# Young768/KungFu

Hardware: AMD Instinct MI355X
Metric: images/sec/GPU ResNet-50 SynchronousSGD at 1/2/4/8 MI355X; scaling efficiency (higher is better)
Workload: dtype bf16

## Files before the change

### csrc/kernels/bind_bn.cpp

```cpp
#include "bind_util.hpp"

#include <vector>

using namespace kfb;

namespace {

const auto kCL = at::MemoryFormat::ChannelsLast;

kfk::BNShape bn_shape(const at::Tensor &x, const char *op) {
    check_cl4(x, op, "x", kAnyGpu);
    const int C = narrow(x.size(1), op, "x");
    TORCH_CHECK(kfk::bn_supported_channels(C), op, ": unsupported channel count ", C);
    return kfk::BNShape{x.numel() / C, C};
}

struct BNCommon {
    float *rm = nullptr, *rv = nullptr;
    int64_t *nbt = nullptr;
};

BNCommon bn_common(const char *op, int C, const Dev &dev, const at::Tensor &weight, const at::Tensor &bias,
                   const OptTensor &running_mean, const OptTensor &running_var, const OptTensor &num_batches,
                   bool training) {
    check_dense(weight, op, "weight", dev, at::kFloat, C);
    check_dense(bias, op, "bias", dev, at::kFloat, C);
    BNCommon b;
    if (has(running_mean)) {
        TORCH_CHECK(has(running_var), op, ": running_var missing");
        b.rm = running_mean->data_ptr<float>();
        b.rv = running_var->data_ptr<float>();
    }
    TORCH_CHECK(training || b.rm, op, ": eval mode needs running stats");
    if (training && has(num_batches)) {
        TORCH_CHECK(num_batches->scalar_type() == at::kLong && num_batches->numel() == 1 && num_batches->is_cuda(),
                    op, ": num_batches_tracked must be a 1-element int64 GPU tensor");
        b.nbt = num_batches->data_ptr<int64_t>();
    }
    return b;
}

at::Tensor bn_dy(at::Tensor dy, const at::Tensor &x, int C, int64_t *ld) {
    *ld = 0;
    if (dy.is_contiguous(kCL)) return dy;
    const int64_t s3 = dy.stride(3);
    const bool slice = dy.stride(1) == 1 && s3 >= C && s3 % 8 == 0 && dy.stride(2) == dy.size(3) * s3 &&
                       dy.stride(0) == dy.size(2) * dy.size(3) * s3 &&
                       reinterpret_cast<uintptr_t>(dy.data_ptr()) % 16 == 0;
    if (!slice) return dy.contiguous(kCL);
    *ld = s3;
    return dy;
}

void check_bn_dy(const at::Tensor &dy, const at::Tensor &x, const char *op) {
    TORCH_CHECK(dy.scalar_type() == at::kBFloat16 && dy.sizes() == x.sizes() && dy.device() == x.device(), op,
                ": dy must be a bf16 tensor of x's shape on its device");
}

std::vector<std::vector<at::Tensor>> bn_finalize_multi(std::vector<at::Tensor> xs, std::vector<at::Tensor> sums,
                                                       std::vector<at::Tensor> weights, std::vector<at::Tensor> biases,
                                                       std::vector<OptTensor> running_means,
                                                       std::vector<OptTensor> running_vars,
                                                       std::vector<OptTensor> num_batches,
                                                       std::vector<double> momentum, std::vector<double> eps) {
    const char *op = "bn_finalize_multi";
    const size_t n = xs.size();
    TORCH_CHECK(n >= 1 && n <= static_cast<size_t>(kfk::kBnFinMax) && sums.size() == n && weights.size() == n &&
                    biases.size() == n && running_means.size() == n && running_vars.size() == n &&
                    num_batches.size() == n && momentum.size() == n && eps.size() == n,
                "bn_finalize_multi: 1..8 BNs, every list of the same length");
    kfk::BnFinBatch b{};
    b.n = static_cast<int>(n);
    for (size_t i = 0; i < n; ++i) {
        auto sh = bn_shape(xs[i], op);
        const Dev dev = xs[0].device();
        TORCH_CHECK(xs[i].device() == *dev, "bn_finalize_multi: xs must be on one device");
        auto c = bn_common(op, sh.channels, dev, weights[i], biases[i], running_means[i], running_vars[i],
                           num_batches[i], true);
        kfk::BnFinDesc &d = b.d[i];
        TORCH_CHECK(sums[i].defined(), "bn_finalize_multi: sums must be defined");
        d.sums = stats_ptr(sums[i], op, sh.channels, dev, "sums");
        d.gamma = weights[i].data_ptr<float>(), d.beta = biases[i].data_ptr<float>();
        d.run_mean = c.rm, d.run_var = c.rv, d.nbt = c.nbt;
        d.rows = sh.rows, d.C = sh.channels;
        d.momentum = static_cast<float>(momentum[i]), d.eps = static_cast<float>(eps[i]);
    }
    std::vector<std::vector<at::Tensor>> out;
    for (size_t i = 0; i < n; ++i) {
        kfk::BnFinDesc &d = b.d[i];
        auto fopt = xs[i].options().dtype(at::kFloat);
        at::Tensor mean = at::empty({d.C}, fopt), invstd = at::empty({d.C}, fopt), coef = at::empty({2 * d.C}, fopt);
        d.mean = mean.data_ptr<float>(), d.invstd = invstd.data_ptr<float>(), d.coef = coef.data_ptr<float>();
        out.push_back({mean, invstd, coef});
    }
    c10::DeviceGuard gd(xs[0].device());
    kfk::launch_bn_sums_finalize_multi(b, stream_of(xs[0], 0));
    return out;
}

std::vector<at::Tensor> bn_forward(at::Tensor x, OptTensor res, at::Tensor weight, at::Tensor bias,
                                   OptTensor running_mean, OptTensor running_var, double momentum, double eps,
                                   bool training, bool relu, OptTensor num_batches, OptTensor sums, OptTensor res_coef,
                                   bool apply, OptTensor out, c10::optional<std::vector<at::Tensor>> pre) {
    const char *op = "bn_forward";
    auto sh = bn_shape(x, op);
    const int C = sh.channels;
    const Dev dev = x.device();
    auto b = bn_common(op, C, dev, weight, bias, running_mean, running_var, num_batches, training);
    const uint16_t *rp = nullptr;
    if (has(res)) {
        check_cl4(*res, op, "res", dev, x.sizes());
        rp = bf16(*res);
    }
    const float *rc = nullptr;
    if (has(res_coef)) {
        TORCH_CHECK(rp, "bn_forward: res_coef (the residual BN's f32 [scale(C); shift(C)]) needs res");
        check_dense(*res_coef, op, "res_coef", dev, at::kFloat, 2 * C);
        rc = res_coef->data_ptr<float>();
    }
    int64_t y_ld = 0;
    if (has(out)) {
        TORCH_CHECK(apply && !rp && relu && out->scalar_type() == at::kBFloat16 && out->sizes() == x.sizes() &&
                        out->stride(1) == 1 && out->stride(3) >= C && out->stride(3) % 8 == 0 &&
                        out->stride(2) == out->size(3) * out->stride(3) &&
                        out->stride(0) == out->size(2) * out->stride(2) &&
                        reinterpret_cast<uintptr_t>(out->data_ptr()) % 16 == 0 && out->device() == x.device(),
                    "bn_forward: out must be a 16-byte aligned channel slice of a channels_last bf16 tensor "
                    "(BN+ReLU, no residual)");
        y_ld = out->stride(3);
    }
    const bool prefin = pre.has_value();
    if (prefin) {
        TORCH_CHECK(pre->size() == 3 && training && has(sums), "bn_forward: pre must be (mean, invstd, coef) with sums");
        check_dense((*pre)[0], op, "pre[0]", dev, at::kFloat, C);
        check_dense((*pre)[1], op, "pre[1]", dev, at::kFloat, C);
        check_dense((*pre)[2], op, "pre[2]", dev, at::kFloat, 2 * C);
    }
    double *sp = training ? stats_ptr(sums, op, C, dev, "sums") : nullptr;

    c10::DeviceGuard gd(x.device());
    auto fopt = x.options().dtype(at::kFloat);
    at::Tensor y;
    if (has(out)) y = *out;
    else if (apply) y = at::empty_like(x, kCL);
    at::Tensor mean, invstd, coef;
    if (prefin) mean = (*pre)[0], invstd = (*pre)[1], coef = (*pre)[2];
    else mean = at::empty({C}, fopt), invstd = at::empty({C}, fopt), coef = at::empty({2 * C}, fopt);
    at::Tensor mask;
    if (apply && rp && relu) mask = at::empty({sh.rows * (C / 8)}, x.options().dtype(at::kByte));
    at::Tensor partial;
    if (training && !sp) partial = at::empty({2 * static_cast<int64_t>(kfk::bn_num_chunks(sh)) * C}, fopt);
    kfk::launch_bn_forward(bf16(x), rp, weight.data_ptr<float>(), bias.data_ptr<float>(),
                           apply ? bf16_mut(y) : nullptr, mask.defined() ? mask.data_ptr<uint8_t>() : nullptr, sh, relu,
                           training, b.rm, b.rv, static_cast<float>(momentum), static_cast<float>(eps),
                           partial.defined() ? partial.data_ptr<float>() : nullptr, mean.data_ptr<float>(),
                           invstd.data_ptr<float>(), coef.data_ptr<float>(), b.nbt, stream_of(x, 0), sp, rc, apply, y_ld,
                           prefin);
    return {y, mean, invstd, coef, mask};
}

std::vector<at::Tensor> bn_backward(at::Tensor dy, at::Tensor x, at::Tensor mean, at::Tensor invstd, at::Tensor weight,
                                    at::Tensor fcoef, OptTensor mask, bool relu, bool training, bool want_dres,
                                    OptTensor sums, OptTensor dres_x, OptTensor dres_sums) {
    const char *op = "bn_backward";
    auto sh = bn_shape(x, op);
    const int C = sh.channels;
    const Dev dev = x.device();
    check_bn_dy(dy, x, op);
    check_dense(mean, op, "mean", dev, at::kFloat, C);
    check_dense(invstd, op, "invstd", dev, at::kFloat, C);
    check_dense(weight, op, "weight", dev, at::kFloat, C);
    check_dense(fcoef, op, "fcoef", dev, at::kFloat, 2 * C);
    const uint8_t *mp = nullptr;
    if (has(mask)) {
        check_dense(*mask, op, "mask", dev, at::kByte, sh.rows * (C / 8));
        mp = mask->data_ptr<uint8_t>();
    }
    double *sp = stats_ptr(sums, op, C, dev, "sums");
    const uint16_t *dsx = nullptr;
    double *dsp = nullptr;
    if (has(dres_x)) {
        TORCH_CHECK(want_dres && has(dres_sums),
                    "bn_backward: dres_x (second BN's input) needs want_dres and its f64 sums workspace dres_sums");
        check_cl4(*dres_x, op, "dres_x", dev, x.sizes());
        dsx = bf16(*dres_x);
        dsp = stats_ptr(dres_sums, op, C, dev, "dres_sums");
    }
    c10::DeviceGuard gd(x.device());
    int64_t dy_ld;
    dy = bn_dy(dy, x, C, &dy_ld);
    auto fopt = x.options().dtype(at::kFloat);
    auto dx = at::empty_like(x, kCL);
    at::Tensor dres;
    if (want_dres) dres = at::empty_like(x, kCL);
    at::Tensor dw = at::empty({C}, fopt), db = at::empty({C}, fopt), coef = at::empty({3 * C}, fopt);
    at::Tensor partial;
    if (!sp) partial = at::empty({2 * static_cast<int64_t>(kfk::bn_num_chunks(sh)) * C}, fopt);
    kfk::launch_bn_backward(bf16(dy), bf16(x), fcoef.data_ptr<float>(), mp, mean.data_ptr<float>(),
                            invstd.data_ptr<float>(), weight.data_ptr<float>(), sh, relu, training,
                            partial.defined() ? partial.data_ptr<float>() : nullptr, dw.data_ptr<float>(),
                            db.data_ptr<float>(), coef.data_ptr<float>(), bf16_mut(dx),
                            want_dres ? bf16_mut(dres) : nullptr, stream_of(x, 0), sp, dsx, dsp, dy_ld);
    return {dx, dres, dw, db};
}

std::vector<std::vector<at::Tensor>> bn_backward_multi(std::vector<at::Tensor> dys, std::vector<at::Tensor> xs,
                                                       std::vector<at::Tensor> means, std::vector<at::Tensor> invstds,
                                                       std::vector<at::Tensor> weights, std::vector<at::Tensor> fcoefs) {
    const char *op = "bn_backward_multi";
    const size_t n = xs.size();
    TORCH_CHECK(n >= 1 && n <= static_cast<size_t>(kfk::kBnFinMax) && dys.size() == n && means.size() == n &&
                    invstds.size() == n && weights.size() == n && fcoefs.size() == n,
                "bn_backward_multi: 1..8 BNs, every list of the same length");
    struct Piece {
        at::Tensor dy, dx, dw, db, coef, partial;
        int64_t ld;
        kfk::BNShape sh;
    };
    std::vector<Piece> ps(n);
    const Dev dev = xs[0].device();
    for (size_t i = 0; i < n; ++i) {
        ps[i].sh = bn_shape(xs[i], op);
        const int C = ps[i].sh.channels;
        TORCH_CHECK(xs[i].device() == *dev, "bn_backward_multi: xs must be on one device");
        check_bn_dy(dys[i], xs[i], op);
        check_dense(fcoefs[i], op, "fcoefs", dev, at::kFloat, 2 * C);
        check_dense(means[i], op, "means", dev, at::kFloat, C);
        check_dense(invstds[i], op, "invstds", dev, at::kFloat, C);
        check_dense(weights[i], op, "weights", dev, at::kFloat, C);
    }
    c10::DeviceGuard gd(xs[0].device());
    kfk::BnBwdFinBatch fb{};
    fb.n = static_cast<int>(n);
    for (size_t i = 0; i < n; ++i) {
        Piece &p = ps[i];
        const int C = p.sh.channels;
        p.dy = bn_dy(dys[i], xs[i], C, &p.ld);
        auto fopt = xs[i].options().dtype(at::kFloat);
        p.dx = at::empty_like(xs[i], kCL);
        p.dw = at::empty({C}, fopt), p.db = at::empty({C}, fopt), p.coef = at::empty({3 * C}, fopt);
        p.partial = at::empty({2 * static_cast<int64_t>(kfk::bn_num_chunks(p.sh)) * C}, fopt);
        kfk::BnBwdFinDesc &d = fb.d[i];
        d.partial = p.partial.data_ptr<float>();
        d.nchunks = kfk::bn_num_chunks(p.sh), d.C = C, d.rows = p.sh.rows;
        d.gamma = weights[i].data_ptr<float>(), d.mean = means[i].data_ptr<float>(), d.invstd = invstds[i].data_ptr<float>();
        d.dgamma = p.dw.data_ptr<float>(), d.dbeta = p.db.data_ptr<float>(), d.coef = p.coef.data_ptr<float>();
    }
    const hipStream_t st = stream_of(xs[0], 0);
    for (int phase : {1, 2}) {
        if (phase == 2) kfk::launch_bn_bwd_finalize_multi(fb, st);
        for (size_t i = 0; i < n; ++i) {
            Piece &p = ps[i];
            kfk::launch_bn_backward(bf16(p.dy), bf16(xs[i]), fcoefs[i].data_ptr<float>(), nullptr,
                                    means[i].data_ptr<float>(), invstds[i].data_ptr<float>(),
                                    weights[i].data_ptr<float>(), p.sh, true, true, p.partial.data_ptr<float>(),
                                    p.dw.data_ptr<float>(), p.db.data_ptr<float>(), p.coef.data_ptr<float>(),
                                    bf16_mut(p.dx), nullptr, st, nullptr, nullptr, nullptr, p.ld, phase);
        }
    }
    std::vector<std::vector<at::Tensor>> out;
    for (auto &p : ps) out.push_back({p.dx, p.dw, p.db});
    return out;
}

std::vector<at::Tensor> bn_pool_forward(at::Tensor x, at::Tensor weight, at::Tensor bias, OptTensor running_mean,
                                        OptTensor running_var, double momentum, double eps, bool training,
                                        OptTensor num_batches, OptTensor sums) {
    const char *op = "bn_pool_forward";
    auto sh = bn_shape(x, op);
    const int C = sh.channels;
    const Dev dev = x.device();
    const int H = narrow(x.size(2), op, "x"), W = narrow(x.size(3), op, "x");
    TORCH_CHECK(kfk::bn_pool_supported(sh, H, W), "bn_pool_forward: unsupported shape");
    double *sp = training ? stats_ptr(sums, op, C, dev, "sums") : nullptr;
    auto b = bn_common(op, C, dev, weight, bias, running_mean, running_var, num_batches, training);
    c10::DeviceGuard gd(x.device());
    auto fopt = x.options().dtype(at::kFloat);
    const int OH = kfk::pool_out(H), OW = kfk::pool_out(W);
    auto yp = at::empty({x.size(0), C, OH, OW}, x.options().memory_format(kCL));
    auto arg = at::empty({x.size(0) * OH * OW * C}, x.options().dtype(at::kByte));
    auto mean = at::empty({C}, fopt), invstd = at::empty({C}, fopt), coef = at::empty({2 * C}, fopt);
    at::Tensor partial, xarg;
    if (training) {
        partial = at::empty({2 * static_cast<int64_t>(kfk::bn_num_chunks(sh)) * C}, fopt);
        xarg = at::empty_like(yp, kCL);
    }
    kfk::launch_bn_pool_forward(bf16(x), weight.data_ptr<float>(), bias.data_ptr<float>(), bf16_mut(yp),
                                arg.data_ptr<uint8_t>(), sh, H, W, training, b.rm, b.rv, static_cast<float>(momentum),
                                static_cast<float>(eps), training ? partial.data_ptr<float>() : nullptr,
                                mean.data_ptr<float>(), invstd.data_ptr<float>(), coef.data_ptr<float>(), b.nbt,
                                stream_of(x, 0), sp, xarg.defined() ? bf16_mut(xarg) : nullptr);
    return {yp, mean, invstd, coef, arg, xarg};
}

std::vector<at::Tensor> bn_pool_backward(at::Tensor dyp, at::Tensor arg, at::Tensor x, at::Tensor mean,
                                         at::Tensor invstd, at::Tensor weight, at::Tensor fcoef, bool training,
                                         OptTensor xarg, bool apply) {
    const char *op = "bn_pool_backward";
    auto sh = bn_shape(x, op);
    const int C = sh.channels;
    const Dev dev = x.device();
    const int H = narrow(x.size(2), op, "x"), W = narrow(x.size(3), op, "x");
    const int64_t psz[4] = {x.size(0), C, kfk::pool_out(H), kfk::pool_out(W)};
    TORCH_CHECK(dyp.scalar_type() == at::kBFloat16 && dyp.sizes() == at::IntArrayRef(psz) && dyp.device() == x.device(),
                "bn_pool_backward: dy must be the pooled [N, C, PH, PW] bf16 gradient on x's device");
    check_dense(arg, op, "arg", dev, at::kByte, dyp.numel());
    check_dense(mean, op, "mean", dev, at::kFloat, C);
    check_dense(invstd, op, "invstd", dev, at::kFloat, C);
    check_dense(weight, op, "weight", dev, at::kFloat, C);
    check_dense(fcoef, op, "fcoef", dev, at::kFloat, 2 * C);
    const bool pooled = training && has(xarg);
    if (pooled) check_cl4(*xarg, op, "xarg", dev, psz);
    c10::DeviceGuard gd(x.device());
    if (!dyp.is_contiguous(kCL)) dyp = dyp.contiguous(kCL);
    auto fopt = x.options().dtype(at::kFloat);
    auto dx = apply ? at::empty_like(x, kCL) : at::empty({0}, x.options());
    auto dw = at::empty({C}, fopt), db = at::empty({C}, fopt), coef = at::empty({3 * C}, fopt);
    auto partial = at::empty({2 * static_cast<int64_t>(kfk::bn_num_chunks(sh)) * C}, fopt);
    at::Tensor sums;
    if (pooled) sums = at::zeros({2 * C * kfk::kStatSlots}, x.options().dtype(at::kDouble));
    kfk::launch_bn_pool_backward(bf16(dyp), arg.data_ptr<uint8_t>(), bf16(x), fcoef.data_ptr<float>(),
                                 mean.data_ptr<float>(), invstd.data_ptr<float>(), weight.data_ptr<float>(), sh, H, W,
                                 training, partial.data_ptr<float>(), dw.data_ptr<float>(), db.data_ptr<float>(),
                                 coef.data_ptr<float>(), apply ? bf16_mut(dx) : nullptr, stream_of(x, 0),
                                 pooled ? bf16(*xarg) : nullptr, pooled ? sums.data_ptr<double>() : nullptr, apply);
    return {dx, dw, db, coef};
}

}

void bind_bn(py::module_ &m) {
    m.def("bn_supported_channels", &kfk::bn_supported_channels);
    m.def("bn_forward", &bn_forward,
          "fused NHWC BN(+residual)(+ReLU) forward -> (y, mean, invstd, coef, relu mask or None)", py::arg("x"),
          py::arg("res"), py::arg("weight"), py::arg("bias"), py::arg("running_mean"), py::arg("running_var"),
          py::arg("momentum"), py::arg("eps"), py::arg("training"), py::arg("relu"),
          py::arg("num_batches") = py::none(), py::arg("sums") = py::none(), py::arg("res_coef") = py::none(),
          py::arg("apply") = true, py::arg("out") = py::none(), py::arg("pre") = py::none());
    m.def("bn_backward_multi", &bn_backward_multi,
          "backward of several BN+ReLUs (slices of one concatenation's gradient): one batched finalize");
    m.def("bn_finalize_multi", &bn_finalize_multi,
          "batched sums-finalize of several training BNs in one launch -> [[mean, invstd, coef], ...]");
    m.def("bn_backward", &bn_backward, "fused NHWC BN(+residual)(+ReLU) backward -> (dx, dres, dweight, dbias)",
          py::arg("dy"), py::arg("x"), py::arg("mean"), py::arg("invstd"), py::arg("weight"), py::arg("fcoef"),
          py::arg("mask"), py::arg("relu"), py::arg("training"), py::arg("want_dres"), py::arg("sums") = py::none(),
          py::arg("dres_x") = py::none(), py::arg("dres_sums") = py::none());
    m.def("bn_pool_supported", [](int64_t C, int64_t H, int64_t W) {
        const char *op = "bn_pool_supported";
        return kfk::bn_pool_supported(kfk::BNShape{H * W, narrow(C, op, "C")}, narrow(H, op, "H"), narrow(W, op, "W"));
    });
    m.def("bn_pool_forward", &bn_pool_forward,
          "stem BN+ReLU+MaxPool(3,2,1) forward -> (y_pool, mean, invstd, coef, argmax)", py::arg("x"),
          py::arg("weight"), py::arg("bias"), py::arg("running_mean"), py::arg("running_var"), py::arg("momentum"),
          py::arg("eps"), py::arg("training"), py::arg("num_batches") = py::none(), py::arg("sums") = py::none());
    m.def("bn_pool_backward", &bn_pool_backward, "stem BN+ReLU+MaxPool backward -> (dx, dweight, dbias, coef)",
          py::arg("dy"), py::arg("arg"), py::arg("x"), py::arg("mean"), py::arg("invstd"), py::arg("weight"),
          py::arg("fcoef"), py::arg("training"), py::arg("xarg") = py::none(), py::arg("apply") = true);
}
```

### csrc/kernels/bn.hip

```cpp
#include "bn_fin.hpp"
#include "common.hpp"
#include "kernels.hpp"

#include <cstdlib>
#include <stdexcept>

namespace kfk {

namespace {

__device__ __forceinline__ void unpack8(const uint4 &v, float (&f)[8]) {
    const uint32_t w[4] = {v.x, v.y, v.z, v.w};
#pragma unroll
    for (int i = 0; i < 4; ++i) {
        f[2 * i] = __uint_as_float(w[i] << 16);
        f[2 * i + 1] = __uint_as_float(w[i] & 0xffff0000u);
    }
}

__device__ __forceinline__ uint4 pack8(const float (&f)[8]) {
    uint32_t w[4];
#pragma unroll
    for (int i = 0; i < 4; ++i)
        w[i] = pack_bf16x2(f[2 * i], f[2 * i + 1]);
    return make_uint4(w[0], w[1], w[2], w[3]);
}

typedef unsigned int kf_u32x4 __attribute__((ext_vector_type(4)));

__device__ __forceinline__ uint4 ld16(const uint4 *p, bool nt) {
    if (nt) {
        const kf_u32x4 v = __builtin_nontemporal_load(reinterpret_cast<const kf_u32x4 *>(p));
        return make_uint4(v.x, v.y, v.z, v.w);
    }
    return *p;
}

__device__ __forceinline__ void st16(uint4 *p, const uint4 &v, bool nt) {
    if (nt) {
        kf_u32x4 w;
        w.x = v.x;
        w.y = v.y;
        w.z = v.z;
        w.w = v.w;
        __builtin_nontemporal_store(w, reinterpret_cast<kf_u32x4 *>(p));
    } else {
        *p = v;
    }
}

int bn_nt_mode() { return 1; }

struct Chunking {
    int64_t rows_per_chunk;
    int nchunks;
};

template <int CVEC>
constexpr int bn_threads() {
    return (kBlock / CVEC) * CVEC;
}

constexpr int kMaxChunks = 512;
constexpr int kFoldCh = 8;
constexpr int kFoldLanes = kBlock / kFoldCh;

template <int NV>
__device__ __forceinline__ void fold_partials(const float *partial, int nchunks, int C, int c, int kl,
                                              double (&out)[NV]) {
    __shared__ double red[NV][kFoldLanes][kFoldCh];
    const int ci = threadIdx.x % kFoldCh;
#pragma unroll
    for (int v = 0; v < NV; ++v) {
        double s = 0;
        if (c < C) {
            const float *p = partial + static_cast<int64_t>(v) * nchunks * C + c;
#pragma unroll 16
            for (int k = kl; k < nchunks; k += kFoldLanes) s += p[static_cast<int64_t>(k) * C];
        }
        red[v][kl][ci] = s;
    }
    __syncthreads();
#pragma unroll
    for (int w = kFoldLanes / 2; w > 0; w >>= 1) {
        if (kl < w) {
#pragma unroll
            for (int v = 0; v < NV; ++v) red[v][kl][ci] += red[v][kl + w][ci];
        }
        __syncthreads();
    }
    if (kl == 0) {
#pragma unroll
        for (int v = 0; v < NV; ++v) out[v] = red[v][0][ci];
    }
}

inline Chunking chunking(const BNShape &sh) {
    const int cvec = sh.channels / 8;
    const int rpi = kBlock / cvec;
    int64_t row_bytes = static_cast<int64_t>(sh.channels) * 2;
    int64_t rpc = (64 * 1024 + row_bytes - 1) / row_bytes;
    rpc = ((rpc + rpi - 1) / rpi) * rpi;
    int64_t n = (sh.rows + rpc - 1) / rpc;
    if (n > kMaxChunks) {
        rpc = (sh.rows + kMaxChunks - 1) / kMaxChunks;
        rpc = ((rpc + rpi - 1) / rpi) * rpi;
        n = (sh.rows + rpc - 1) / rpc;
    }
    if (n < 1) n = 1;
    return {rpc, static_cast<int>(n)};
}

template <int CVEC, int NV>
__device__ __forceinline__ void reduce_to_partials(float (&acc)[NV][8], float *lds, float *partial, int C,
                                                   int nchunks_total) {
    constexpr int RPI = kBlock / CVEC;
    const int tid = threadIdx.x, cv = tid % CVEC, r0 = tid / CVEC;
#pragma unroll
    for (int v = 0; v < NV; ++v) {
        float *dst = lds + (v * RPI + r0) * C + cv * 8;
#pragma unroll
        for (int k = 0; k < 8; ++k) dst[k] = acc[v][k];
    }
    __syncthreads();
    for (int c = tid; c < C; c += bn_threads<CVEC>()) {
#pragma unroll
        for (int v = 0; v < NV; ++v) {
            float s = 0.f;
#pragma unroll
            for (int r = 0; r < RPI; ++r) s += lds[(v * RPI + r) * C + c];
            partial[(static_cast<int64_t>(v) * nchunks_total + blockIdx.x) * C + c] = s;
        }
    }
}


template <int CVEC>
__global__ __launch_bounds__(kBlock) void bn_stats_kernel(const uint4 *__restrict__ x, int64_t rows,
                                                          int64_t rows_per_chunk, float *partial) {
    constexpr int RPI = kBlock / CVEC;
    constexpr int C = CVEC * 8;
    __shared__ float lds[2 * RPI * C];
    const int tid = threadIdx.x, cv = tid % CVEC, r0 = tid / CVEC;
    float acc[2][8];
#pragma unroll
    for (int k = 0; k < 8; ++k) acc[0][k] = acc[1][k] = 0.f;
    const int64_t r_begin = static_cast<int64_t>(blockIdx.x) * rows_per_chunk;
    int64_t r_end = r_begin + rows_per_chunk;
    if (r_end > rows) r_end = rows;
    int64_t r = r_begin + r0;
    for (; r + 3 * RPI < r_end; r += 4 * RPI) {
        uint4 v[4];
#pragma unroll
        for (int u = 0; u < 4; ++u) v[u] = x[(r + u * RPI) * CVEC + cv];
#pragma unroll
        for (int u = 0; u < 4; ++u) {
            float f[8];
            unpack8(v[u], f);
#pragma unroll
            for (int k = 0; k < 8; ++k) {
                acc[0][k] += f[k];
                acc[1][k] += f[k] * f[k];
            }
        }
    }
    for (; r < r_end; r += RPI) {
        float f[8];
        unpack8(x[r * CVEC + cv], f);
#pragma unroll
        for (int k = 0; k < 8; ++k) {
            acc[0][k] += f[k];
            acc[1][k] += f[k] * f[k];
        }
    }
    reduce_to_partials<CVEC, 2>(acc, lds, partial, C, gridDim.x);
}

__global__ __launch_bounds__(kBlock) void bn_stats_finalize(const float *partial, int nchunks, int C, int64_t rows,
                                                            const float *gamma, const float *beta, float *mean,
                                                            float *invstd, float *run_mean, float *run_var,
                                                            float momentum, float eps, float *coef,
                                                            int64_t *num_batches) {
    const int c = blockIdx.x * kFoldCh + threadIdx.x % kFoldCh, kl = threadIdx.x / kFoldCh;
    double sums[2];
    fold_partials<2>(partial, nchunks, C, c, kl, sums);
    if (num_batches && blockIdx.x == 0 && threadIdx.x == 0) num_batches[0] += 1;
    if (kl != 0 || c >= C) return;
    double s = sums[0], q = sums[1];
    double m = s / rows;
    double var = q / rows - m * m;
    if (var < 0) var = 0;
    float is = rsqrtf(static_cast<float>(var) + eps);
    mean[c] = static_cast<float>(m);
    invstd[c] = is;
    if (run_mean) {
        double unbiased = rows > 1 ? var * rows / (rows - 1) : var;
        run_mean[c] = (1.f - momentum) * run_mean[c] + momentum * static_cast<float>(m);
        run_var[c] = (1.f - momentum) * run_var[c] + momentum * static_cast<float>(unbiased);
    }
    float g = gamma ? gamma[c] : 1.f, b = beta ? beta[c] : 0.f;
    float sc = g * is;
    coef[c] = sc;
    coef[C + c] = b - static_cast<float>(m) * sc;
}

__global__ __launch_bounds__(256) void bn_sums_finalize(double *__restrict__ sums, int C, int64_t rows,
                                                        const float *__restrict__ gamma,
                                                        const float *__restrict__ beta, float *mean, float *invstd,
                                                        float *run_mean, float *run_var, float momentum, float eps,
                                                        float *coef, int64_t *num_batches) {
    const int c = blockIdx.x * blockDim.x + threadIdx.x;
    if (num_batches && c == 0) num_batches[0] += 1;
    if (c >= C) return;
    const float g = gamma ? gamma[c] : 1.f, b = beta ? beta[c] : 0.f;
    const float rm = run_mean ? run_mean[c] : 0.f, rv = run_mean ? run_var[c] : 0.f;
    const double *sp = sums + c;
    double vs[kStatSlots], vq[kStatSlots];
#pragma unroll
    for (int k = 0; k < kStatSlots; ++k) {
        vs[k] = sp[k * 2 * C];
        vq[k] = sp[k * 2 * C + C];
    }
    double s = 0, q = 0;
#pragma unroll
    for (int k = 0; k < kStatSlots; ++k) {
        s += vs[k];
        q += vq[k];
    }
    double *zp = sums + c;
#pragma unroll
    for (int k = 0; k < kStatSlots; ++k) {
        zp[k * 2 * C] = 0.0;
        zp[k * 2 * C + C] = 0.0;
    }
    bn_fin_fwd_channel(c, C, s, q, rows, g, b, rm, rv, mean, invstd, run_mean, run_var, momentum, eps, coef);
}

__global__ __launch_bounds__(256) void bn_sums_finalize_multi(BnFinBatch b) {
    const BnFinDesc &d = b.d[blockIdx.y];
    const int c = blockIdx.x * blockDim.x + threadIdx.x;
    if (d.nbt && c == 0) d.nbt[0] += 1;
    if (c >= d.C) return;
    const int C = d.C;
    const float g = d.gamma ? d.gamma[c] : 1.f, bb = d.beta ? d.beta[c] : 0.f;
    const float rm = d.run_mean ? d.run_mean[c] : 0.f, rv = d.run_mean ? d.run_var[c] : 0.f;
    const double *sp = d.sums + c;
    double vs[kStatSlots], vq[kStatSlots];
#pragma unroll
    for (int k = 0; k < kStatSlots; ++k) {
        vs[k] = sp[k * 2 * C];
        vq[k] = sp[k * 2 * C + C];
    }
    double s = 0, q = 0;
#pragma unroll
    for (int k = 0; k < kStatSlots; ++k) {
        s += vs[k];
        q += vq[k];
    }
    double *zp = d.sums + c;
#pragma unroll
    for (int k = 0; k < kStatSlots; ++k) {
        zp[k * 2 * C] = 0.0;
        zp[k * 2 * C + C] = 0.0;
    }
    bn_fin_fwd_channel(c, C, s, q, d.rows, g, bb, rm, rv, d.mean, d.invstd, d.run_mean, d.run_var, d.momentum, d.eps,
                       d.coef);
}

__global__ void bn_eval_coef(int C, const float *gamma, const float *beta, const float *run_mean,
                             const float *run_var, float eps, float *mean, float *invstd, float *coef) {
    int c = blockIdx.x * blockDim.x + threadIdx.x;
    if (c >= C) return;
    float is = rsqrtf(run_var[c] + eps);
    float g = gamma ? gamma[c] : 1.f, b = beta ? beta[c] : 0.f;
    mean[c] = run_mean[c];
    invstd[c] = is;
    coef[c] = g * is;
    coef[C + c] = b - run_mean[c] * g * is;
}


template <int CVEC, bool RES, bool RELU, bool RESC = false, bool SOUT = false>
__global__ __launch_bounds__(kBlock) void bn_apply_kernel(const uint4 *__restrict__ x, const uint4 *__restrict__ res,
                                                          const float *__restrict__ coef, uint4 *__restrict__ y,
                                                          uint8_t *__restrict__ mask, int64_t nvec,
                                                          const float *__restrict__ rcoef = nullptr, int ntm = 0,
                                                          int64_t y_ldv = 0) {
    constexpr int C = CVEC * 8;
    const bool ntl = ntm & 1, nts = ntm & 2;
    const int64_t tid = static_cast<int64_t>(blockIdx.x) * bn_threads<CVEC>() + threadIdx.x;
    const int cv = static_cast<int>(tid % CVEC);
    float sc[8], sh[8], rsc[8], rsh[8];
#pragma unroll
    for (int k = 0; k < 8; ++k) {
        sc[k] = coef[cv * 8 + k];
        sh[k] = coef[C + cv * 8 + k];
        if (RESC) {
            rsc[k] = rcoef[cv * 8 + k];
            sh[k] += rcoef[C + cv * 8 + k];
        }
    }
    const int64_t stride = static_cast<int64_t>(gridDim.x) * bn_threads<CVEC>();
    constexpr int U = 2;
    for (int64_t i0 = tid; i0 < nvec; i0 += U * stride) {
        uint4 xr[U], rr4[U];
#pragma unroll
        for (int u = 0; u < U; ++u) {
            const int64_t i = i0 + u * stride;
            if (i < nvec) {
                xr[u] = ld16(x + i, ntl);
                if (RES) rr4[u] = ld16(res + i, ntl);
            }
        }
#pragma unroll
        for (int u = 0; u < U; ++u) {
            const int64_t i = i0 + u * stride;
            if (i >= nvec) break;
            float f[8];
            unpack8(xr[u], f);
            float rr[8];
            if (RES) unpack8(rr4[u], rr);
            uint32_t m = 0;
#pragma unroll
            for (int k = 0; k < 8; ++k) {
                float v = f[k] * sc[k] + sh[k];
                if (RESC) v += rr[k] * rsc[k];
                else if (RES) v += rr[k];
                if (RELU) {
                    m |= (v > 0.f ? 1u : 0u) << k;
                    v = v > 0.f ? v : 0.f;
                }
                f[k] = v;
            }
            if constexpr (SOUT) st16(y + (i / CVEC) * y_ldv + cv, pack8(f), nts);
            else st16(y + i, pack8(f), nts);
            if (RES && RELU) mask[i] = static_cast<uint8_t>(m);
        }
    }
}


template <int CVEC>
__global__ __launch_bounds__(kBlock) void bn_pool_apply_kernel(const uint4 *__restrict__ x,
                                                               const float *__restrict__ coef, uint4 *__restrict__ yp,
                                                               uint2 *__restrict__ arg, int H, int W, int OH, int OW,
                                                               int64_t nout_vec, uint4 *__restrict__ xarg) {
    constexpr int C = CVEC * 8;
    const int64_t tid = static_cast<int64_t>(blockIdx.x) * bn_threads<CVEC>() + threadIdx.x;
    const int cv = static_cast<int>(tid % CVEC);
    float sc[8], sh[8];
#pragma unroll
    for (int k = 0; k < 8; ++k) {
        sc[k] = coef[cv * 8 + k];
        sh[k] = coef[C + cv * 8 + k];
    }
    const int64_t stride = static_cast<int64_t>(gridDim.x) * bn_threads<CVEC>();
    for (int64_t i = tid; i < nout_vec; i += stride) {
        const int64_t p = i / CVEC;
        const int ow = static_cast<int>(p % OW);
        const int64_t t = p / OW;
        const int oh = static_cast<int>(t % OH);
        const int64_t n = t / OH;
        float best[8], xb[8];
        uint32_t a[8];
#pragma unroll
        for (int k = 0; k < 8; ++k) {
            best[k] = -1.f;
            a[k] = 0;
            xb[k] = 0.f;
        }
#pragma unroll
        for (int kh = 0; kh < 3; ++kh) {
            const int h = 2 * oh - 1 + kh;
            if (h < 0 || h >= H) continue;
#pragma unroll
            for (int kw = 0; kw < 3; ++kw) {
                const int w = 2 * ow - 1 + kw;
                if (w < 0 || w >= W) continue;
                float f[8];
                unpack8(x[((n * H + h) * W + w) * CVEC + cv], f);
#pragma unroll
                for (int k = 0; k < 8; ++k) {
                    float v = f[k] * sc[k] + sh[k];
                    v = v > 0.f ? v : 0.f;
                    if (v > best[k]) {
                        best[k] = v;
                        a[k] = kh * 3 + kw;
                        xb[k] = f[k];
                    }
                }
            }
        }
        yp[i] = pack8(best);
        arg[i] = make_uint2(a[0] | (a[1] << 8) | (a[2] << 16) | (a[3] << 24),
                            a[4] | (a[5] << 8) | (a[6] << 16) | (a[7] << 24));
        if (xarg) xarg[i] = pack8(xb);
    }
}

template <int CVEC>
__global__ __launch_bounds__(kBlock) void bn_pool_bwd_sums_kernel(const uint4 *__restrict__ dy,
                                                                  const uint4 *__restrict__ xarg,
                                                                  const float *__restrict__ fcoef,
                                                                  double *__restrict__ sums, int64_t nvec) {
    constexpr int C = CVEC * 8, NT = bn_threads<CVEC>();
    const int64_t tid = static_cast<int64_t>(blockIdx.x) * NT + threadIdx.x;
    const int cv = static_cast<int>(tid % CVEC);
    float sc[8], sh[8], s1[8], s2[8];
#pragma unroll
    for (int k = 0; k < 8; ++k) {
        sc[k] = fcoef[cv * 8 + k];
        sh[k] = fcoef[C + cv * 8 + k];
        s1[k] = s2[k] = 0.f;
    }
    const int64_t stride = static_cast<int64_t>(gridDim.x) * NT;
    for (int64_t i = tid; i < nvec; i += stride) {
        float g[8], xv[8];
        unpack8(dy[i], g);
        unpack8(xarg[i], xv);
#pragma unroll
        for (int k = 0; k < 8; ++k) {
            const float dz = xv[k] * sc[k] + sh[k] > 0.f ? g[k] : 0.f;
            s1[k] += dz;
            s2[k] += dz * xv[k];
        }
    }
    __shared__ float red[kBlock][17];
    if (threadIdx.x < NT) {
#pragma unroll
        for (int k = 0; k < 8; ++k) {
            red[threadIdx.x][k] = s1[k];
            red[threadIdx.x][8 + k] = s2[k];
        }
    }
    __syncthreads();
    for (int c = threadIdx.x; c < C; c += NT) {
        const int cvi = c >> 3, k = c & 7;
        double a1 = 0, a2 = 0;
        for (int u = cvi; u < NT; u += CVEC) {
            a1 += red[u][k];
            a2 += red[u][8 + k];
        }
        double *sl = sums + (blockIdx.x % kStatSlots) * 2 * C;
        atomicAdd(sl + c, a1);
        atomicAdd(sl + C + c, a2);
    }
}


struct DirectGrad {
    const uint4 *dy;
    bool nt = false;
    using Raw = uint4;
    template <int CVEC>
    __device__ __forceinline__ Raw fetch(int64_t i, int64_t , int ) const {
        return ld16(dy + i, nt);
    }
    __device__ __forceinline__ void get(const Raw &r, float (&g)[8]) const { unpack8(r, g); }
};

struct StridedGrad {
    const uint4 *dy;
    int64_t ldv;
    using Raw = uint4;
    template <int CVEC>
    __device__ __forceinline__ Raw fetch(int64_t , int64_t row, int cv) const {
        return dy[row * ldv + cv];
    }
    __device__ __forceinline__ void get(const Raw &r, float (&g)[8]) const { unpack8(r, g); }
};

struct PoolGrad {
    const uint4 *dyp;
    const uint2 *arg;
    int H, W, OH, OW;
    uint64_t m_hw, m_w;
    struct Raw {
        uint2 am[4];
        uint4 d[4];
        uint32_t kk;
    };
    __device__ __forceinline__ void get(const Raw &r, float (&g)[8]) const {
#pragma unroll
        for (int k = 0; k < 8; ++k) g[k] = 0.f;
#pragma unroll
        for (int c = 0; c < 4; ++c) {
            const uint32_t kk = (r.kk >> (8 * c)) & 0xffu;
            float d[8];
            unpack8(r.d[c], d);
#pragma unroll
            for (int k = 0; k < 8; ++k) {
                const uint32_t ak = ((k < 4 ? r.am[c].x : r.am[c].y) >> (8 * (k & 3))) & 0xffu;
                g[k] += ak == kk ? d[k] : 0.f;
            }
        }
    }
    template <int CVEC>
    __device__ __forceinline__ Raw fetch(int64_t , int64_t row64, int cv) const {
        const uint32_t row = static_cast<uint32_t>(row64);
        const uint32_t hw = static_cast<uint32_t>(H) * static_cast<uint32_t>(W);
        const uint32_t n = static_cast<uint32_t>((static_cast<uint64_t>(row) * m_hw) >> 40);
        const uint32_t rem = row - n * hw;
        const int h = static_cast<int>((static_cast<uint64_t>(rem) * m_w) >> 40);
        const int w = static_cast<int>(rem) - h * W;
        const int oh_lo = h >> 1, oh_hi = (h + 1) >> 1;
        const int ow_lo = w >> 1, ow_hi = (w + 1) >> 1;
        Raw r;
        r.kk = 0;
        const uint32_t base = (n * OH) * OW;
#pragma unroll
        for (int c = 0; c < 4; ++c) {
            const int oh = (c & 2) ? oh_hi : oh_lo, ow = (c & 1) ? ow_hi : ow_lo;
            const bool ok = (!(c & 2) || oh_hi != oh_lo) && (!(c & 1) || ow_hi != ow_lo) && oh < OH && ow < OW;
            const uint32_t kk = ok ? static_cast<uint32_t>((h + 1 - 2 * oh) * 3 + (w + 1 - 2 * ow)) : 0xffu;
            const uint32_t o = ((base + (ok ? oh : oh_lo) * OW + (ok ? ow : ow_lo)) * CVEC) + cv;
            r.am[c] = arg[o];
            r.d[c] = dyp[o];
            r.kk |= kk << (8 * c);
        }
        return r;
    }
    template <int CVEC>
    __device__ __forceinline__ void load(int64_t i, int64_t row, int cv, float (&g)[8]) const {
        get(fetch<CVEC>(i, row, cv), g);
    }
};

enum ReluMode : int { RM_NONE = 0, RM_COEF = 1, RM_BITS = 2 };

template <int RM>
__device__ __forceinline__ void relu_gate(float (&g)[8], const float (&xv)[8], const float (&sc)[8],
                                          const float (&sh)[8], const uint8_t *mask, int64_t i) {
    if (RM == RM_COEF) {
#pragma unroll
        for (int k = 0; k < 8; ++k) g[k] = (xv[k] * sc[k] + sh[k]) > 0.f ? g[k] : 0.f;
    } else if (RM == RM_BITS) {
        const uint32_t m = mask[i];
#pragma unroll
        for (int k = 0; k < 8; ++k) g[k] = ((m >> k) & 1u) ? g[k] : 0.f;
    }
}

template <int CVEC, int RM>
__device__ __forceinline__ void load_fwd_coef(const float *fcoef, int cv, float (&sc)[8], float (&sh)[8]) {
    constexpr int C = CVEC * 8;
#pragma unroll
    for (int k = 0; k < 8; ++k) {
        sc[k] = RM == RM_COEF ? fcoef[cv * 8 + k] : 0.f;
        sh[k] = RM == RM_COEF ? fcoef[C + cv * 8 + k] : 0.f;
    }
}


template <int CVEC, int RM, class G>
__global__ __launch_bounds__(kBlock) void bn_bwd_reduce_kernel(G grad, const uint4 *__restrict__ x,
                                                               const float *__restrict__ fcoef,
                                                               const uint8_t *__restrict__ mask, int64_t rows,
                                                               int64_t rows_per_chunk, float *partial, int ntm = 0) {
    const bool ntl = ntm & 1;
    constexpr int RPI = kBlock / CVEC;
    constexpr int C = CVEC * 8;
    __shared__ float lds[2 * RPI * C];
    const int tid = threadIdx.x, cv = tid % CVEC, r0 = tid / CVEC;
    float sc[8], sh[8];
    load_fwd_coef<CVEC, RM>(fcoef, cv, sc, sh);
    float acc[2][8];
#pragma unroll
    for (int k = 0; k < 8; ++k) acc[0][k] = acc[1][k] = 0.f;
    const int64_t r_begin = static_cast<int64_t>(blockIdx.x) * rows_per_chunk;
    int64_t r_end = r_begin + rows_per_chunk;
    if (r_end > rows) r_end = rows;
    int64_t r = r_begin + r0;
    constexpr int U = 4;
    for (; r + (U - 1) * RPI < r_end; r += U * RPI) {
        typename G::Raw gr[U];
        uint4 xr[U];
#pragma unroll
        for (int u = 0; u < U; ++u) {
            const int64_t row = r + u * RPI, i = row * CVEC + cv;
            gr[u] = grad.template fetch<CVEC>(i, row, cv);
            xr[u] = ld16(x + i, ntl);
        }
#pragma unroll
        for (int u = 0; u < U; ++u) {
            float g[8], xv[8];
            grad.get(gr[u], g);
            unpack8(xr[u], xv);
            relu_gate<RM>(g, xv, sc, sh, mask, (r + u * RPI) * CVEC + cv);
#pragma unroll
            for (int k = 0; k < 8; ++k) {
                acc[0][k] += g[k];
                acc[1][k] += g[k] * xv[k];
            }
        }
    }
    for (; r < r_end; r += RPI) {
        const int64_t i = r * CVEC + cv;
        float g[8], xv[8];
        grad.get(grad.template fetch<CVEC>(i, r, cv), g);
        unpack8(x[i], xv);
        relu_gate<RM>(g, xv, sc, sh, mask, i);
#pragma unroll
        for (int k = 0; k < 8; ++k) {
            acc[0][k] += g[k];
            acc[1][k] += g[k] * xv[k];
        }
    }
    reduce_to_partials<CVEC, 2>(acc, lds, partial, C, gridDim.x);
}

__global__ __launch_bounds__(kBlock) void bn_bwd_finalize(const float *partial, int nchunks, int C, int64_t rows,
                                                          const float *gamma, const float *mean, const float *invstd,
                                                          float *dgamma, float *dbeta, float *coef, bool training) {
    const int c = blockIdx.x * kFoldCh + threadIdx.x % kFoldCh, kl = threadIdx.x / kFoldCh;
    double sums[2];
    fold_partials<2>(partial, nchunks, C, c, kl, sums);
    if (kl != 0 || c >= C) return;
    double db = sums[0], dg = static_cast<double>(invstd[c]) * (sums[1] - static_cast<double>(mean[c]) * db);
    dgamma[c] = static_cast<float>(dg);
    dbeta[c] = static_cast<float>(db);
    float g = gamma ? gamma[c] : 1.f;
    float a = g * invstd[c];
    if (training) {
        float inv_m = 1.f / static_cast<float>(rows);
        float k2 = -a * static_cast<float>(dg) * invstd[c] * inv_m;
        coef[c] = a;
        coef[C + c] = k2;
        coef[2 * C + c] = -a * static_cast<float>(db) * inv_m - k2 * mean[c];
    } else {
        coef[c] = a;
        coef[C + c] = 0.f;
        coef[2 * C + c] = 0.f;
    }
}

__global__ __launch_bounds__(kBlock) void bn_bwd_finalize_multi(BnBwdFinBatch b) {
    const BnBwdFinDesc &d = b.d[blockIdx.y];
    const int C = d.C;
    if (static_cast<int>(blockIdx.x) * kFoldCh >= C) return;
    const int c = blockIdx.x * kFoldCh + threadIdx.x % kFoldCh, kl = threadIdx.x / kFoldCh;
    double sums[2];
    fold_partials<2>(d.partial, d.nchunks, C, c, kl, sums);
    if (kl != 0 || c >= C) return;
    double db = sums[0], dg = static_cast<double>(d.invstd[c]) * (sums[1] - static_cast<double>(d.mean[c]) * db);
    d.dgamma[c] = static_cast<float>(dg);
    d.dbeta[c] = static_cast<float>(db);
    float g = d.gamma ? d.gamma[c] : 1.f;
    float a = g * d.invstd[c];
    const float inv_m = 1.f / static_cast<float>(d.rows);
    const float k2 = -a * static_cast<float>(dg) * d.invstd[c] * inv_m;
    d.coef[c] = a;
    d.coef[C + c] = k2;
    d.coef[2 * C + c] = -a * static_cast<float>(db) * inv_m - k2 * d.mean[c];
}

__global__ __launch_bounds__(256) void bn_bwd_finalize_sums(double *__restrict__ sums, int C, int64_t rows,
                                                            const float *__restrict__ gamma,
                                                            const float *__restrict__ mean,
                                                            const float *__restrict__ invstd, float *dgamma,
                                                            float *dbeta, float *coef, bool training) {
    const int c = blockIdx.x * blockDim.x + threadIdx.x;
    if (c >= C) return;
    const float g = gamma ? gamma[c] : 1.f, mu = mean[c], is = invstd[c];
    const double *sp = sums + c;
    double v0[kStatSlots], v1[kStatSlots];
#pragma unroll
    for (int k = 0; k < kStatSlots; ++k) {
        v0[k] = sp[k * 2 * C];
        v1[k] = sp[k * 2 * C + C];
    }
    double s0 = 0, s1 = 0;
#pragma unroll
    for (int k = 0; k < kStatSlots; ++k) {
        s0 += v0[k];
        s1 += v1[k];
    }
    double *zp = sums + c;
#pragma unroll
    for (int k = 0; k < kStatSlots; ++k) {
        zp[k * 2 * C] = 0.0;
        zp[k * 2 * C + C] = 0.0;
    }
    bn_fin_bwd_channel(c, C, s0, s1, rows, g, mu, is, dgamma, dbeta, coef, training);
}


template <int CVEC, int RM, bool DRES, class G>
__global__ __launch_bounds__(kBlock) void bn_bwd_apply_kernel(G grad, const uint4 *__restrict__ x,
                                                              const float *__restrict__ fcoef,
                                                              const uint8_t *__restrict__ mask,
                                                              const float *__restrict__ coef, uint4 *__restrict__ dx,
                                                              uint4 *__restrict__ dres, int64_t nvec,
                                                              const uint4 *__restrict__ dsx = nullptr,
                                                              double *__restrict__ dsums = nullptr, int ntm = 0) {
    constexpr int C = CVEC * 8;
    const bool ntl = ntm & 1, nts = ntm & 2;
    const int64_t tid = static_cast<int64_t>(blockIdx.x) * bn_threads<CVEC>() + threadIdx.x;
    const int cv = static_cast<int>(tid % CVEC);
    float k1[8], k2[8], k3[8], sc[8], sh[8];
#pragma unroll
    for (int k = 0; k < 8; ++k) {
        k1[k] = coef[cv * 8 + k];
        k2[k] = coef[C + cv * 8 + k];
        k3[k] = coef[2 * C + cv * 8 + k];
    }
    load_fwd_coef<CVEC, RM>(fcoef, cv, sc, sh);
    float d1[8], d2[8];
#pragma unroll
    for (int k = 0; k < 8; ++k) d1[k] = d2[k] = 0.f;
    const bool dsum = DRES && dsx != nullptr;
    const int64_t stride = static_cast<int64_t>(gridDim.x) * bn_threads<CVEC>();
    constexpr int U = 2;
    for (int64_t i0 = tid; i0 < nvec; i0 += U * stride) {
        typename G::Raw gr[U];
        uint4 xr[U];
#pragma unroll
        for (int u = 0; u < U; ++u) {
            const int64_t i = i0 + u * stride;
            if (i < nvec) {
                gr[u] = grad.template fetch<CVEC>(i, i / CVEC, cv);
                xr[u] = ld16(x + i, ntl);
            }
        }
#pragma unroll
        for (int u = 0; u < U; ++u) {
            const int64_t i = i0 + u * stride;
            if (i >= nvec) break;
            float g[8], xv[8];
            grad.get(gr[u], g);
            unpack8(xr[u], xv);
            relu_gate<RM>(g, xv, sc, sh, mask, i);
            if (DRES) {
                const uint4 gr = pack8(g);
                st16(dres + i, gr, nts);
                if (dsum) {
                    float gq[8], sx[8];
                    unpack8(gr, gq);
                    unpack8(dsx[i], sx);
#pragma unroll
                    for (int k = 0; k < 8; ++k) {
                        d1[k] += gq[k];
                        d2[k] += gq[k] * sx[k];
                    }
                }
            }
            float o[8];
#pragma unroll
            for (int k = 0; k < 8; ++k) o[k] = k1[k] * g[k] + k2[k] * xv[k] + k3[k];
            st16(dx + i, pack8(o), nts);
        }
    }
    if (dsum) {
        constexpr int NT = bn_threads<CVEC>();
        __shared__ float red[kBlock][17];
        if (threadIdx.x < NT) {
#pragma unroll
            for (int k = 0; k < 8; ++k) {
                red[threadIdx.x][k] = d1[k];
                red[threadIdx.x][8 + k] = d2[k];
            }
        }
        __syncthreads();
        for (int c = threadIdx.x; c < C; c += NT) {
            const int cvi = c >> 3, k = c & 7;
            double a1 = 0, a2 = 0;
            for (int u = cvi; u < NT; u += CVEC) {
                a1 += red[u][k];
                a2 += red[u][8 + k];
            }
            double *sl = dsums + (blockIdx.x % kStatSlots) * 2 * C;
            atomicAdd(sl + c, a1);
            atomicAdd(sl + C + c, a2);
        }
    }
}

template <typename F>
void dispatch_cvec(int cvec, F &&f) {
    switch (cvec) {
    case 4: f(std::integral_constant<int, 4>()); break;
    case 6: f(std::integral_constant<int, 6>()); break;
    case 10: f(std::integral_constant<int, 10>()); break;
    case 12: f(std::integral_constant<int, 12>()); break;
    case 20: f(std::integral_constant<int, 20>()); break;
    case 24: f(std::integral_constant<int, 24>()); break;
    case 40: f(std::integral_constant<int, 40>()); break;
    case 48: f(std::integral_constant<int, 48>()); break;
    case 56: f(std::integral_constant<int, 56>()); break;
    case 8: f(std::integral_constant<int, 8>()); break;
    case 16: f(std::integral_constant<int, 16>()); break;
    case 32: f(std::integral_constant<int, 32>()); break;
    case 64: f(std::integral_constant<int, 64>()); break;
    case 128: f(std::integral_constant<int, 128>()); break;
    case 256: f(std::integral_constant<int, 256>()); break;
    default: break;
    }
}

int apply_grid(int64_t nvec, int cvec) {
    const int nt = (kBlock / cvec) * cvec;
    int64_t g = (nvec + nt - 1) / nt;
    if (g > kMaxGrid) g = kMaxGrid;
    if (g < 1) g = 1;
    return static_cast<int>(g);
}

void launch_stats(const uint16_t *x, BNShape sh, const float *gamma, const float *beta, float *run_mean,
                  float *run_var, float momentum, float eps, float *partial, float *mean, float *invstd, float *coef,
                  int64_t *num_batches, hipStream_t s) {
    const int C = sh.channels, cvec = C / 8;
    Chunking ch = chunking(sh);
    dispatch_cvec(cvec, [&](auto cvc) {
        constexpr int CV = decltype(cvc)::value;
        bn_stats_kernel<CV><<<ch.nchunks, bn_threads<CV>(), 0, s>>>(reinterpret_cast<const uint4 *>(x), sh.rows,
                                                          ch.rows_per_chunk, partial);
    });
    bn_stats_finalize<<<(C + kFoldCh - 1) / kFoldCh, kBlock, 0, s>>>(partial, ch.nchunks, C, sh.rows, gamma, beta,
                                                                     mean, invstd, run_mean, run_var, momentum, eps,
                                                                     coef, num_batches);
}

template <class G>
void launch_backward_impl(G grad, const uint16_t *x, const float *fcoef, const uint8_t *mask, const float *mean,
                          const float *invstd, const float *gamma, BNShape sh, int rm, bool training, float *partial,
                          float *dgamma, float *dbeta, float *coef, uint16_t *dx, uint16_t *dres, hipStream_t s,
                          double *sums = nullptr, const uint16_t *dres_x = nullptr, double *dres_sums = nullptr,
                          int phase = 0) {
    const int C = sh.channels, cvec = C / 8;
    const int64_t nvec = sh.rows * cvec;
    Chunking ch = chunking(sh);
    const uint4 *xx = reinterpret_cast<const uint4 *>(x);
    if (phase == 2) {
    } else if (sums) {
        bn_bwd_finalize_sums<<<(C + 255) / 256, 256, 0, s>>>(sums, C, sh.rows, gamma, mean, invstd, dgamma, dbeta,
                                                             coef, training);
    } else {
    dispatch_cvec(cvec, [&](auto cvc) {
        constexpr int CV = decltype(cvc)::value;
        auto go = [&](auto rmc) {
            constexpr int RM = decltype(rmc)::value;
            bn_bwd_reduce_kernel<CV, RM, G>
                <<<ch.nchunks, bn_threads<CV>(), 0, s>>>(grad, xx, fcoef, mask, sh.rows, ch.rows_per_chunk, partial,
                                                          bn_nt_mode());
        };
        if (rm == RM_COEF) go(std::integral_constant<int, RM_COEF>());
        else if (rm == RM_BITS) go(std::integral_constant<int, RM_BITS>());
        else go(std::integral_constant<int, RM_NONE>());
    });
    if (phase == 1) return;
    bn_bwd_finalize<<<(C + kFoldCh - 1) / kFoldCh, kBlock, 0, s>>>(partial, ch.nchunks, C, sh.rows, gamma, mean,
                                                                   invstd, dgamma, dbeta, coef, training);
    }
    if (phase == 3) return;
    const int g = apply_grid(nvec, cvec);
    uint4 *o = reinterpret_cast<uint4 *>(dx), *r = reinterpret_cast<uint4 *>(dres);
    dispatch_cvec(cvec, [&](auto cvc) {
        constexpr int CV = decltype(cvc)::value;
        auto go = [&](auto rmc, auto drc) {
            constexpr int RM = decltype(rmc)::value;
            constexpr bool DR = decltype(drc)::value;
            bn_bwd_apply_kernel<CV, RM, DR, G><<<g, bn_threads<CV>(), 0, s>>>(
                grad, xx, fcoef, mask, coef, o, r, nvec, DR ? reinterpret_cast<const uint4 *>(dres_x) : nullptr,
                DR ? dres_sums : nullptr, bn_nt_mode());
        };
        using T = std::true_type;
        using F = std::false_type;
        if (rm == RM_COEF) {
            if (dres) go(std::integral_constant<int, RM_COEF>(), T());
            else go(std::integral_constant<int, RM_COEF>(), F());
        } else if (rm == RM_BITS) {
            if (dres) go(std::integral_constant<int, RM_BITS>(), T());
            else go(std::integral_constant<int, RM_BITS>(), F());
        } else {
            if (dres) go(std::integral_constant<int, RM_NONE>(), T());
            else go(std::integral_constant<int, RM_NONE>(), F());
        }
    });
}

}

void launch_bn_bwd_finalize_multi(const BnBwdFinBatch &b, hipStream_t s) {
    if (b.n <= 0) return;
    if (b.n > kBnFinMax) throw std::invalid_argument("bn_bwd_finalize_multi: too many BNs");
    int cmax = 0;
    for (int i = 0; i < b.n; ++i) cmax = b.d[i].C > cmax ? b.d[i].C : cmax;
    bn_bwd_finalize_multi<<<dim3((cmax + kFoldCh - 1) / kFoldCh, b.n), kBlock, 0, s>>>(b);
}

void launch_bn_sums_finalize_multi(const BnFinBatch &b, hipStream_t s) {
    if (b.n <= 0) return;
    if (b.n > kBnFinMax) throw std::invalid_argument("bn_sums_finalize_multi: too many BNs");
    int cmax = 0;
    for (int i = 0; i < b.n; ++i) cmax = b.d[i].C > cmax ? b.d[i].C : cmax;
    bn_sums_finalize_multi<<<dim3((cmax + 255) / 256, b.n), 256, 0, s>>>(b);
}

bool bn_supported_channels(int C) {
    if (C % 8) return false;
    switch (C / 8) {
    case 4: case 6: case 8: case 10: case 12: case 16: case 20: case 24: case 32: case 40: case 48: case 56:
    case 64: case 128: case 256:
        return true;
    default:
        return false;
    }
}

int bn_num_chunks(BNShape sh) { return chunking(sh).nchunks; }

void launch_bn_forward(const uint16_t *x, const uint16_t *res, const float *gamma, const float *beta, uint16_t *y,
                       uint8_t *mask, BNShape sh, bool relu, bool training, float *run_mean, float *run_var,
                       float momentum, float eps, float *partial, float *mean, float *invstd, float *coef,
                       int64_t *num_batches, hipStream_t s, double *sums, const float *res_coef, bool apply,
                       int64_t y_ld, bool prefinalized) {
    const int C = sh.channels, cvec = C / 8;
    if (y_ld > 0 && (y_ld % 8 || y_ld < C || res || !relu))
        throw std::invalid_argument("bn_forward: a strided output needs BN+ReLU without residual, row stride % 8");
    const int64_t nvec = sh.rows * cvec;
    if (training && sums) {
        if (!prefinalized)
            bn_sums_finalize<<<(C + 255) / 256, 256, 0, s>>>(sums, C, sh.rows, gamma, beta, mean, invstd, run_mean,
                                                             run_var, momentum, eps, coef, num_batches);
    } else if (training) {
        launch_stats(x, sh, gamma, beta, run_mean, run_var, momentum, eps, partial, mean, invstd, coef, num_batches,
                     s);
    } else {
        bn_eval_coef<<<(C + 255) / 256, 256, 0, s>>>(C, gamma, beta, run_mean, run_var, eps, mean, invstd, coef);
    }
    if (!apply) return;
    const int g = apply_grid(nvec, cvec);
    const int ntm = bn_nt_mode();
    dispatch_cvec(cvec, [&](auto cvc) {
        constexpr int CV = decltype(cvc)::value;
        constexpr int NT = bn_threads<CV>();
        const uint4 *xv = reinterpret_cast<const uint4 *>(x);
        const uint4 *rv = reinterpret_cast<const uint4 *>(res);
        uint4 *yv = reinterpret_cast<uint4 *>(y);
        if (res && res_coef) {
            if (relu) bn_apply_kernel<CV, true, true, true><<<g, NT, 0, s>>>(xv, rv, coef, yv, mask, nvec, res_coef, ntm);
            else bn_apply_kernel<CV, true, false, true><<<g, NT, 0, s>>>(xv, rv, coef, yv, mask, nvec, res_coef, ntm);
        } else if (res) {
            if (relu) bn_apply_kernel<CV, true, true><<<g, NT, 0, s>>>(xv, rv, coef, yv, mask, nvec, nullptr, ntm);
            else bn_apply_kernel<CV, true, false><<<g, NT, 0, s>>>(xv, rv, coef, yv, mask, nvec, nullptr, ntm);
        } else if (y_ld > 0 && y_ld != C) {
            bn_apply_kernel<CV, false, true, false, true><<<g, NT, 0, s>>>(xv, rv, coef, yv, mask, nvec, nullptr, ntm,
                                                                          y_ld / 8);
        } else {
            if (relu) bn_apply_kernel<CV, false, true><<<g, NT, 0, s>>>(xv, rv, coef, yv, mask, nvec, nullptr, ntm);
            else bn_apply_kernel<CV, false, false><<<g, NT, 0, s>>>(xv, rv, coef, yv, mask, nvec, nullptr, ntm);
        }
    });
}

void launch_bn_backward(const uint16_t *dy, const uint16_t *x, const float *fcoef, const uint8_t *mask,
                        const float *mean, const float *invstd, const float *gamma, BNShape sh, bool relu,
                        bool training, float *partial, float *dgamma, float *dbeta, float *coef, uint16_t *dx,
                        uint16_t *dres, hipStream_t s, double *sums, const uint16_t *dres_x, double *dres_sums,
                        int64_t dy_ld, int phase) {
    const int rm = !relu ? RM_NONE : (mask ? RM_BITS : RM_COEF);
    if (dy_ld > 0 && dy_ld != sh.channels) {
        if (dy_ld % 8) throw std::invalid_argument("bn_backward: dy row stride must be a multiple of 8");
        launch_backward_impl(StridedGrad{reinterpret_cast<const uint4 *>(dy), dy_ld / 8}, x, fcoef, mask, mean, invstd,
                             gamma, sh, rm, training, partial, dgamma, dbeta, coef, dx, dres, s, sums, dres_x,
                             dres_sums, phase);
        return;
    }
    launch_backward_impl(DirectGrad{reinterpret_cast<const uint4 *>(dy), (bn_nt_mode() & 1) != 0}, x, fcoef, mask, mean, invstd, gamma, sh, rm,
                         training, partial, dgamma, dbeta, coef, dx, dres, s, sums, dres_x, dres_sums, phase);
}

bool bn_pool_supported(BNShape sh, int H, int W) {
    return bn_supported_channels(sh.channels) && H >= 2 && W >= 2 && sh.rows % (static_cast<int64_t>(H) * W) == 0 &&
           sh.rows * (sh.channels / 8) < (int64_t(1) << 31);
}

void launch_bn_pool_forward(const uint16_t *x, const float *gamma, const float *beta, uint16_t *yp, uint8_t *arg,
                            BNShape sh, int H, int W, bool training, float *run_mean, float *run_var, float momentum,
                            float eps, float *partial, float *mean, float *invstd, float *coef, int64_t *num_batches,
                            hipStream_t s, double *sums, uint16_t *xarg) {
    const int C = sh.channels, cvec = C / 8;
    if (training && sums) {
        bn_sums_finalize<<<(C + 255) / 256, 256, 0, s>>>(sums, C, sh.rows, gamma, beta, mean, invstd, run_mean,
                                                         run_var, momentum, eps, coef, num_batches);
    } else if (training) {
        launch_stats(x, sh, gamma, beta, run_mean, run_var, momentum, eps, partial, mean, invstd, coef, num_batches,
                     s);
    } else {
        bn_eval_coef<<<(C + 255) / 256, 256, 0, s>>>(C, gamma, beta, run_mean, run_var, eps, mean, invstd, coef);
    }
    const int OH = pool_out(H), OW = pool_out(W);
    const int64_t N = sh.rows / (static_cast<int64_t>(H) * W);
    const int64_t nout = N * OH * OW * cvec;
    const int g = apply_grid(nout, cvec);
    dispatch_cvec(cvec, [&](auto cvc) {
        constexpr int CV = decltype(cvc)::value;
        bn_pool_apply_kernel<CV><<<g, bn_threads<CV>(), 0, s>>>(reinterpret_cast<const uint4 *>(x), coef,
                                                      reinterpret_cast<uint4 *>(yp), reinterpret_cast<uint2 *>(arg), H,
                                                      W, OH, OW, nout, reinterpret_cast<uint4 *>(xarg));
    });
}

void launch_bn_pool_backward(const uint16_t *dyp, const uint8_t *arg, const uint16_t *x, const float *fcoef,
                             const float *mean, const float *invstd, const float *gamma, BNShape sh, int H, int W,
                             bool training, float *partial, float *dgamma, float *dbeta, float *coef, uint16_t *dx,
                             hipStream_t s, const uint16_t *xarg, double *sums, bool apply) {
    if (xarg && sums && training) {
        const int C = sh.channels, cvec = C / 8;
        const int64_t nvec = sh.rows / (static_cast<int64_t>(H) * W) * pool_out(H) * pool_out(W) * cvec;
        const int g = apply_grid(nvec, cvec);
        dispatch_cvec(cvec, [&](auto cvc) {
            constexpr int CV = decltype(cvc)::value;
            bn_pool_bwd_sums_kernel<CV><<<g, bn_threads<CV>(), 0, s>>>(
                reinterpret_cast<const uint4 *>(dyp), reinterpret_cast<const uint4 *>(xarg), fcoef, sums, nvec);
        });
    } else {
        sums = nullptr;
    }
    const uint64_t m_hw = (uint64_t(1) << 40) / (static_cast<uint64_t>(H) * W) + 1;
    const uint64_t m_w = (uint64_t(1) << 40) / static_cast<uint64_t>(W) + 1;
    if (static_cast<uint64_t>(sh.rows) * H * W >= (uint64_t(1) << 40))
        throw std::invalid_argument("bn_pool_backward: too many rows for the 40-bit division");
    PoolGrad pg{reinterpret_cast<const uint4 *>(dyp), reinterpret_cast<const uint2 *>(arg), H, W, pool_out(H),
                pool_out(W), m_hw, m_w};
    launch_backward_impl(pg, x, fcoef, nullptr, mean, invstd, gamma, sh, RM_COEF, training, partial, dgamma, dbeta,
                         coef, dx, nullptr, s, sums, nullptr, nullptr, apply ? 0 : 3);
}

}
```

### csrc/kernels/bn_fin.hpp

```cpp
#pragma once

#include <hip/hip_runtime.h>

#include <cstdint>

namespace kfk {

__device__ __forceinline__ void bn_fin_fwd_channel(int c, int C, double s, double q, int64_t rows, float g, float b,
                                                   float rm, float rv, float *mean, float *invstd, float *run_mean,
                                                   float *run_var, float momentum, float eps, float *coef) {
    const double m = s / rows;
    double var = q / rows - m * m;
    if (var < 0) var = 0;
    const float is = rsqrtf(static_cast<float>(var) + eps);
    const float sc = g * is;
    mean[c] = static_cast<float>(m);
    invstd[c] = is;
    if (run_mean) {
        const double unbiased = rows > 1 ? var * rows / (rows - 1) : var;
        run_mean[c] = (1.f - momentum) * rm + momentum * static_cast<float>(m);
        run_var[c] = (1.f - momentum) * rv + momentum * static_cast<float>(unbiased);
    }
    coef[c] = sc;
    coef[C + c] = b - static_cast<float>(m) * sc;
}

__device__ __forceinline__ void bn_fin_bwd_channel(int c, int C, double s0, double s1, int64_t rows, float g,
                                                   float mu, float is, float *dgamma, float *dbeta, float *coef,
                                                   bool training) {
    const double db = s0, dg = static_cast<double>(is) * (s1 - static_cast<double>(mu) * db);
    dgamma[c] = static_cast<float>(dg);
    dbeta[c] = static_cast<float>(db);
    const float a = g * is;
    if (training) {
        const float inv_m = 1.f / static_cast<float>(rows);
        const float k2 = -a * static_cast<float>(dg) * is * inv_m;
        coef[c] = a;
        coef[C + c] = k2;
        coef[2 * C + c] = -a * static_cast<float>(db) * inv_m - k2 * mu;
    } else {
        coef[c] = a;
        coef[C + c] = 0.f;
        coef[2 * C + c] = 0.f;
    }
}

}
```

### csrc/kernels/kernels.hpp

```cpp
#pragma once

#include <hip/hip_runtime.h>

#include <cstddef>
#include <cstdint>
#include <string>
#include <vector>

namespace kfk {

constexpr int kMaxGridHost = 2048;

void launch_reduce(void *z, const void *x, const void *y, size_t n, int dtype, int op, hipStream_t s);

void launch_embedding_backward(float *grad, const int64_t *ids, const void *dy, bool dy_bf16, int64_t T, int D,
                               int64_t V, hipStream_t s, int ch = 0);

void set_dropout_seed_base(const uint32_t *p);
const uint32_t *dropout_seed_base();

constexpr int kGemmBias = 1, kGemmAccum = 2, kGemmGeluGrad = 4;
bool gemm_nt_supported(int64_t M, int64_t N, int64_t K);
int gemm_nt_pick_bn(int64_t M, int64_t N);
void launch_gemm_nt(const uint16_t *a, const uint16_t *b, uint16_t *c, const uint16_t *bias, int M, int N, int K,
                    int epi, int bn, hipStream_t s);
bool gemm_nt_ld_supported(int64_t M, int64_t N, int64_t K, int64_t ldc);
void launch_gemm_nt_ld(const uint16_t *a, const uint16_t *b, uint16_t *c, const uint16_t *bias, int M, int N, int K,
                       int ldc, int epi, int bn, hipStream_t s);
int gemm_nt_gelu_grad_rows(int M);
void launch_gemm_nt_gelu_grad(const uint16_t *a, const uint16_t *b, uint16_t *c, const uint16_t *u, float *part, int M,
                              int N, int K, hipStream_t s);
void launch_colsum_fold(const float *part, int rows, int O, float *out_f32, uint16_t *out_bf16, hipStream_t s);

void launch_comm_emulate(const void *bucket, void *scratch, int64_t bytes, int64_t traffic_bytes, int ctas,
                         double seconds, hipStream_t s);

void launch_sgd(float *w, const float *g, float *m, uint16_t *shadow, size_t n, float lr, const float *lr_dev,
                float mu, float damp, float wd, float gscale, bool nesterov, bool first, hipStream_t s);

void launch_adam(float *w, const float *g, float *m, float *v, size_t n, float lr, const float *lr_dev, float b1,
                 float b2, float eps, float wd, bool adamw, float gscale, const float *step_dev, hipStream_t s,
                 uint16_t *shadow = nullptr);

void launch_axpby(void *y, const void *x, void *z, size_t n, float a, float b, int dtype, hipStream_t s);

void launch_scale(void *x, size_t n, float alpha, int dtype, hipStream_t s);

void launch_square(float *dst, const void *src, size_t n, int dtype, hipStream_t s);
void launch_cast(void *dst, const void *src, size_t n, int src_dt, int dst_dt, float scale, hipStream_t s);

int colsum_chunks(int64_t T, int O);
void launch_colsum_bf16(const uint16_t *x, int64_t T, int O, float *part, float *out_f32, uint16_t *out_bf16,
                        hipStream_t s);
int gelu_colsum_chunks(int64_t T, int O);
class PairPrefetcher {
  public:
    struct Job {
        uintptr_t pending_ev = 0;
        int64_t pending_ver = 0;
        uintptr_t host_copy = 0;
        int target = 0;
        std::vector<uintptr_t> src_slots;
        int64_t own_ver = 0;
        uintptr_t dst = 0;
        uintptr_t after_ev = 0;
        uintptr_t host_stage = 0;
    };
    struct Result {
        int status = 0;
        int64_t version = 0, own_ver = 0;
        std::string error;
    };
    PairPrefetcher(const std::string &libpath, int device, int self_rank, const std::string &rec_name,
                   const std::string &model_name, int64_t nbytes, int slots);
    ~PairPrefetcher();
    PairPrefetcher(const PairPrefetcher &) = delete;
    PairPrefetcher &operator=(const PairPrefetcher &) = delete;
    void start(const Job &job);
    bool busy();
    Result finish(uintptr_t wait_stream);

  private:
    struct Impl;
    Impl *d_;
};

void launch_xent_forward(const uint16_t *x, const int64_t *labels, int64_t R, int V, float *lse, float *loss,
                         hipStream_t s, int64_t ld = 0);
void launch_xent_backward(const uint16_t *x, const int64_t *labels, const float *lse, const float *scale, int64_t R,
                          int V, uint16_t *dx, hipStream_t s, int64_t ld = 0);

void launch_gelu_bwd_colsum(const uint16_t *dy, const uint16_t *u, uint16_t *du, int64_t T, int O, float *part,
                            float *out_f32, uint16_t *out_bf16, hipStream_t s);
void launch_sumsq2(const void *a, const void *b, size_t n, int dtype, float *partials, float *out, hipStream_t s);

void launch_variance(const float *s1, const float *s2, size_t n, float inv_np, float *partials, float *out,
                     hipStream_t s);

void launch_seg_variance(const float *s1, const float *s2, size_t n, float inv_np, const int64_t *seg_off, int nseg,
                         float *out, hipStream_t s);

void launch_gns_update(const float *sumsq_small, const float *sumsq_big, float b_small, float b_big, float alpha,
                       float *state, hipStream_t s);

void launch_pack(const int64_t *desc, int n_tensors, size_t total, void *flat, int flat_dtype, int src_dtype,
                 float scale, hipStream_t s);
void launch_unpack(const int64_t *desc, int n_tensors, size_t total, const void *flat, int flat_dtype,
                   int dst_dtype, float scale, hipStream_t s);

struct GradAccTable {
    static constexpr int kMax = 48;
    int n = 0;
    int src_dtype = 0;
    float scale = 1.f;
    const void *src[kMax];
    int64_t off[kMax];
    int64_t numel[kMax];
    int blk_start[kMax + 1];
};
int grad_accumulate_blocks(int64_t numel);
void launch_grad_accumulate(const GradAccTable &tab, float *flat, hipStream_t s);

constexpr int kStatSlots = 16;
bool conv_supported(int Cin, int Cout, int ks, int stride);
int conv_variants();
enum ConvEpi : int {
    kEpiFwdStats = 1, kEpiAccum = 2, kEpiBwdCoef = 4, kEpiBwdBits = 8, kEpiBiasRelu = 16, kEpiGate = 32,
    kEpiAccMask = 64, kEpiAccEven = 128, kEpiBias = 256, kEpiGeluGrad = 1024
};
struct EpiArgs {
    const uint8_t *amask = nullptr;
    const uint16_t *bias = nullptr;
    double *stats = nullptr;
    const uint16_t *bx = nullptr;
    const float *fcoef = nullptr;
    const uint8_t *bmask = nullptr;
};
void launch_conv(const uint16_t *x, const uint16_t *w, uint16_t *y, int N, int H, int W, int Cin, int Cout, int ks,
                 int stride, const EpiArgs &ea, int epi, hipStream_t s, int variant = -1);
void launch_conv_dgrad_s2(const uint16_t *dy, const uint16_t *wt, uint16_t *dx, int N, int OH, int OW, int Cout,
                          int Cin, int ks, const EpiArgs &ea, int epi, hipStream_t s, int variant = -1, int DH = 0,
                          int DW = 0, int pad = 1);
bool gemm_supported(int M, int K, int N);
void launch_gemm(const uint16_t *x, const uint16_t *w, uint16_t *y, int M, int K, int N, const EpiArgs &ea, int epi,
                 hipStream_t s, int variant = -1);
bool conv_rect_supported(int Cin, int Cout, int kh, int kw, int stride);
void launch_conv_rect(const uint16_t *x, const uint16_t *w, uint16_t *y, int N, int H, int W, int Cin, int Cout,
                      int kh, int kw, int ph, int pw, int stride, const EpiArgs &ea, int epi, hipStream_t s);
struct FlipTable {
    static constexpr int kMax = 64;
    int n = 0;
    const uint16_t *src[kMax];
    uint16_t *dst[kMax];
    int cout[kMax], cin[kMax], taps[kMax];
    int64_t start[kMax + 1];
    int tstart[kMax + 1];
};
void launch_conv_flip_multi(const FlipTable &tab, hipStream_t s);
void launch_conv_flip_weight(const uint16_t *w, uint16_t *wt, int Cout, int Cin, int ks, hipStream_t s);
void launch_conv_flip_weight_taps(const uint16_t *w, uint16_t *wt, int Cout, int Cin, int taps, hipStream_t s);

struct WgradPlan {
    int variant = 0;
    int splits = 1;
    int kps = 0;
    int64_t ws_floats = 0;
};
bool conv_wgrad_supported(int Cin, int Cout, int ks, int stride);
int64_t conv_wgrad_max_pixels(int N, int H, int W, int Cin, int Cout, int ks, int stride);
WgradPlan conv_wgrad_plan(int N, int H, int W, int Cin, int Cout, int ks, int stride, int variant = -1,
                          int splits = -1);
void launch_conv_wgrad(const uint16_t *dy, const uint16_t *x, void *dw, float *part, int N, int H, int W, int Cin,
                       int Cout, int ks, int stride, const WgradPlan &plan, bool out_f32, bool accumulate,
                       hipStream_t s, bool atomics = true);
bool conv_wgrad_rect_supported(int Cin, int Cout, int kh, int kw, int stride);
WgradPlan conv_wgrad_rect_plan(int N, int H, int W, int Cin, int Cout, int kh, int kw, int ph, int pw, int stride,
                               int variant = -1);
int conv_wgrad_rows_rect_auto(int N, int H, int W, int Cin, int Cout, int kh, int kw, int ph, int pw, int stride);
bool conv_wgrad_rows_rect_supported(int N, int H, int W, int Cin, int Cout, int kh, int kw, int ph, int pw,
                                    int stride);
void launch_conv_wgrad_rect(const uint16_t *dy, const uint16_t *x, void *dw, float *part, int N, int H, int W,
                            int Cin, int Cout, int kh, int kw, int ph, int pw, int stride, const WgradPlan &plan,
                            bool out_f32, bool accumulate, hipStream_t s);
int conv_wgrad_variants();

void launch_stem_pad4(const uint16_t *x, uint16_t *x4, int64_t npix, hipStream_t s);
void launch_stem_pad4_f32(const float *x, uint16_t *x4, int64_t npix, hipStream_t s);
void launch_stem_pack_weight(const uint16_t *w, uint16_t *wp, hipStream_t s);
int stem_out(int h);
int stem3_out(int h, int k, int stride, int pad);
void launch_stem3_pack_weight(const uint16_t *w, uint16_t *wp, int Cout, int KH, int KW, hipStream_t s);
void launch_stem3_forward(const void *x, bool x_f32, const uint16_t *wp, uint16_t *y, double *stats, const float *bias,
                          bool relu, int Cout, int N, int H, int W, int KH, int KW, int stride, int ph, int pw,
                          hipStream_t s);
int stem3_wgrad_blocks(int Cout, int N, int H, int W, int KH, int KW, int stride, int ph, int pw);
int64_t stem3_wgrad_workspace(int Cout, int N, int H, int W, int KH, int KW, int stride, int ph, int pw);
void launch_stem3_wgrad(const uint16_t *dy, const void *x, bool x_f32, void *dw, bool out_f32, float *part, int Cout,
                        int N, int H, int W, int KH, int KW, int stride, int ph, int pw, hipStream_t s);
void launch_stem_forward(const uint16_t *x4, const uint16_t *wp, uint16_t *y, double *stats, int N, int H, int W,
                         hipStream_t s);
int stem_wgrad_splits(int N, int H, int W);
int64_t stem_wgrad_workspace(int N, int H, int W, int splits);
bool stem_wgrad_bnp_supported(int N, int H, int W);
void launch_stem_wgrad_bnp(const uint16_t *y, const uint16_t *x4, uint16_t *dw, float *part, int N, int H, int W,
                           int splits, const uint16_t *dyp, const uint8_t *arg, const float *fcoef,
                           const float *bcoef, hipStream_t s);
void launch_stem_wgrad(const uint16_t *dy, const uint16_t *x4, uint16_t *dw, float *part, int N, int H, int W,
                       int splits, hipStream_t s);

struct BNShape {
    int64_t rows;
    int channels;
};
bool bn_supported_channels(int C);
int bn_num_chunks(BNShape sh);
struct BnFinDesc {
    double *sums;
    const float *gamma, *beta;
    float *mean, *invstd, *run_mean, *run_var, *coef;
    int64_t *nbt;
    int64_t rows;
    int C;
    float momentum, eps;
};
constexpr int kBnFinMax = 8;
struct BnFinBatch {
    BnFinDesc d[kBnFinMax];
    int n;
};
void launch_bn_sums_finalize_multi(const BnFinBatch &b, hipStream_t s);
struct BnBwdFinDesc {
    const float *partial;
    int nchunks, C;
    int64_t rows;
    const float *gamma, *mean, *invstd;
    float *dgamma, *dbeta, *coef;
};
struct BnBwdFinBatch {
    BnBwdFinDesc d[kBnFinMax];
    int n;
};
void launch_bn_bwd_finalize_multi(const BnBwdFinBatch &b, hipStream_t s);

void launch_bn_forward(const uint16_t *x, const uint16_t *res, const float *gamma, const float *beta, uint16_t *y,
                       uint8_t *mask, BNShape sh, bool relu, bool training, float *run_mean, float *run_var,
                       float momentum, float eps, float *partial, float *mean, float *invstd, float *coef,
                       int64_t *num_batches, hipStream_t s, double *sums = nullptr, const float *res_coef = nullptr,
                       bool apply = true, int64_t y_ld = 0, bool prefinalized = false);
void launch_bn_backward(const uint16_t *dy, const uint16_t *x, const float *fcoef, const uint8_t *mask,
                        const float *mean, const float *invstd, const float *gamma, BNShape sh, bool relu,
                        bool training, float *partial, float *dgamma, float *dbeta, float *coef, uint16_t *dx,
                        uint16_t *dres, hipStream_t s, double *sums = nullptr, const uint16_t *dres_x = nullptr,
                        double *dres_sums = nullptr, int64_t dy_ld = 0, int phase = 0);

inline int pool_out(int h) { return (h + 2 - 3) / 2 + 1; }
bool bn_pool_supported(BNShape sh, int H, int W);
void launch_bn_pool_forward(const uint16_t *x, const float *gamma, const float *beta, uint16_t *yp, uint8_t *arg,
                            BNShape sh, int H, int W, bool training, float *run_mean, float *run_var, float momentum,
                            float eps, float *partial, float *mean, float *invstd, float *coef, int64_t *num_batches,
                            hipStream_t s, double *sums = nullptr, uint16_t *xarg = nullptr);
void launch_bn_pool_backward(const uint16_t *dyp, const uint8_t *arg, const uint16_t *x, const float *fcoef,
                             const float *mean, const float *invstd, const float *gamma, BNShape sh, int H, int W,
                             bool training, float *partial, float *dgamma, float *dbeta, float *coef, uint16_t *dx,
                             hipStream_t s, const uint16_t *xarg = nullptr, double *sums = nullptr, bool apply = true);

bool bias_act_supported(int C);
void launch_bias_act_forward(uint16_t *y, const float *bias, int64_t rows, int C, bool relu, hipStream_t s);
int bias_act_backward_blocks(int64_t rows, int C);
void launch_bias_act_backward(const uint16_t *dy, const uint16_t *y, uint16_t *dz, float *dbias, float *partial,
                              int64_t rows, int C, bool relu, hipStream_t s);

void launch_maxpool2x2_forward(const uint16_t *x, uint16_t *y, int64_t N, int H, int W, int C, hipStream_t s);
int maxpool3s2_out(int h, int pad);
void launch_maxpool3s2_forward(const uint16_t *x, uint16_t *y, uint8_t *arg, int64_t N, int H, int W, int C, int pad,
                               hipStream_t s);
void launch_maxpool3s2_backward(const uint16_t *dy, const uint8_t *arg, uint16_t *dx, int64_t N, int H, int W, int C,
                                int pad, hipStream_t s);
void launch_avgpool3s1(const uint16_t *x, uint16_t *y, int64_t N, int H, int W, int C, hipStream_t s);
void launch_global_avgpool_forward(const uint16_t *x, uint16_t *y, int64_t N, int HW, int C, hipStream_t s);
void launch_global_avgpool_backward(const uint16_t *dy, uint16_t *dx, int64_t N, int HW, int C, hipStream_t s);

bool layernorm_supported(int D);
int layernorm_bwd_blocks(int64_t rows);
void launch_layernorm_forward(const uint16_t *x, const uint16_t *r, const float *gamma, const float *beta, uint16_t *y,
                              uint16_t *s, float *mean, float *rstd, int64_t rows, int D, float eps, hipStream_t st,
                              float p = 0.f, uint32_t seed = 0);
void launch_layernorm_backward(const uint16_t *dy, const uint16_t *s, const float *gamma, const float *mean,
                               const float *rstd, uint16_t *ds, float *partial, float *dgamma, float *dbeta,
                               int64_t rows, int D, hipStream_t st,
                               uint16_t *dr = nullptr, float p = 0.f, uint32_t seed = 0, float *rb_f32 = nullptr,
                               uint16_t *rb_bf16 = nullptr);
void launch_maxpool2x2_backward(const uint16_t *x, const uint16_t *dy, uint16_t *dx, int64_t N, int H, int W, int C,
                                hipStream_t s, double *gate_stats = nullptr);

bool attention_supported(int S, int head_dim);
void launch_attention_forward(const uint16_t *qkv, uint16_t *out, float *lse, int B, int S, int H, float scale,
                              uint32_t seed, float p_drop, hipStream_t s);
void launch_attention_backward(const uint16_t *qkv, const uint16_t *out, const float *lse, const uint16_t *dout,
                               uint16_t *dqkv, int B, int S, int H, float scale, uint32_t seed, float p_drop,
                               hipStream_t s);

}
```

### kungfu_amd/knobs.py

```python
from __future__ import annotations

import difflib
import os
import warnings
from typing import Dict, NamedTuple, Optional


class Knob(NamedTuple):
    default: Optional[str]
    kind: str
    doc: str


class KnobWarning(UserWarning):
    pass


def _u(default, doc):
    return Knob(default, "user", doc)


def _l(doc):
    return Knob(None, "launcher", doc)


def _t(default, doc):
    return Knob(default, "test", doc)


def _d(default, doc):
    return Knob(default, "dev", doc)


KNOBS: Dict[str, Knob] = {
    "KUNGFU_CONFIG_LOG_LEVEL": _u("INFO", "runtime log level (DEBUG/INFO/WARN/ERROR)"),
    "KUNGFU_CONFIG_ENABLE_MONITORING": _u("false", "net monitor + /metrics endpoint"),
    "KUNGFU_CONFIG_MONITORING_PERIOD": _u("1s", "net monitor sampling period"),
    "KUNGFU_CONFIG_ENABLE_STALL_DETECTION": _u("false", "log host collectives that take > 10 s"),
    "KUNGFU_CONFIG_ENABLE_TRACE": _u("false", "print trace-scope reports at exit"),
    "KUNGFU_CONFIG_CHUNK_SIZE_MIB": _u("1", "host all-reduce chunk size (strategies rotate per chunk)"),
    "KUNGFU_CONFIG_STRATEGY_HASH_METHOD": _u("SIMPLE", "chunk -> strategy assignment (SIMPLE | NAME)"),
    "KUNGFU_CONFIG_CONN_RETRY_COUNT": _u("500", "TCP dial retries"),
    "KUNGFU_CONFIG_CONN_RETRY_PERIOD": _u("200ms", "TCP dial retry period"),
    "KUNGFU_CONFIG_USE_UNIX_SOCK": _u("true", "same-host peers over Unix sockets"),
    "KUNGFU_CONFIG_WAIT_RUNNER_TIMEOUT": _u("120s", "elastic: wait for a runner"),
    "KUNGFU_CONFIG_RETRY_STDERR_PREFIX": _u(None, "runner restarts a worker whose stderr starts with this"),
    "KUNGFU_ALLREDUCE_STRATEGY": _u("AUTO", "host all-reduce topology strategy"),
    "KUNGFU_OP_TIMEOUT_S": _u("0", "host collective watchdog: abort (exit 3) after this many seconds; 0 = off"),
    "KUNGFU_MNIST_DIR": _u(None, "MNIST idx files for the examples"),
    "KUNGFU_PLATFORM": _u(None, "launcher platform hint (ModelArts discovery)"),
    "KUNGFU_GPU_DATAPLANE": _u("rccl", "rccl | host (stage device collectives through host memory)"),
    "KUNGFU_GPU_ALLREDUCE": _u("rccl", "rccl | graph (bucket all-reduce along the KungFu strategy graphs)"),
    "KUNGFU_BUCKET_MB": _u("32", "S-SGD gradient bucket size (MiB)"),
    "KUNGFU_TAIL_BUCKET_MB": _u("4", "size cap of the buckets holding the first layers (exposed tail)"),
    "KUNGFU_RCCL_TIMEOUT_S": _u("600", "RCCL watchdog stall timeout; setting it explicitly makes a stall fatal"),
    "KUNGFU_RCCL_STALL_ACTION": _u("log", "log | abort: what a stalled RCCL collective does"),
    "KUNGFU_RCCL_INIT_TIMEOUT_S": _u("300", "communicator init / finalize deadline"),
    "KUNGFU_RCCL_BLOCKING": _u("0", "1: blocking communicator init (no deadline, no CTA budget)"),
    "KUNGFU_RCCL_MIN_CTAS": _u("0", "ncclConfig_t.minCTAs (0 = RCCL default); _<SCOPE> suffix per scope"),
    "KUNGFU_RCCL_MAX_CTAS": _u("0", "ncclConfig_t.maxCTAs (0 = RCCL default); _<SCOPE> suffix per scope"),
    "KUNGFU_NATIVE_BACKTRACE": _u("0", "1: print a native backtrace on SIGSEGV/SIGBUS/SIGABRT (debugging)"),
    "KUNGFU_RCCL_COLOCATE": _t("0", "1: several RCCL ranks on one GPU (socket transport; tests)"),
    "KUNGFU_COMM_EMULATE": _u(None, "ranks=R,ctas=C,busbw=GB/s,lat_us=L: model an R-rank all-reduce on one GPU"),
    "KUNGFU_PREFLIGHT_TIMEOUT_S": _u("60", "bench pre-flight: deadline of each device check"),
    "KUNGFU_PREFLIGHT_CORRUPT": _t(None, "test hook: this rank corrupts its pre-flight buffer"),
    "KUNGFU_PREFLIGHT_CORRUPT_WHAT": _t("ipc", "test hook: ipc | allreduce | stall (reports a stall without stalling)"),
    "KUNGFU_FORCE_DEVICE": _t(None, "pin every rank to this HIP device (colocated tests)"),
    "KUNGFU_INIT_CKPT": _u(None, "elastic: initial checkpoint step"),
    "KUNGFU_CONV3X3": _u("1", "3x3 convolutions on the MFMA kernel"),
    "KUNGFU_CONV_RECT": _u("1", "rectangular-window convolutions on the MFMA kernel"),
    "KUNGFU_WGRAD": _u("1", "weight gradients on the split-K MFMA kernel"),
    "KUNGFU_WGRAD_RECT": _u("1", "rectangular-window weight gradients on the MFMA kernels"),
    "KUNGFU_FUSED_BLOCK": _u("1", "ResNet bottleneck as one fused autograd node"),
    "KUNGFU_STEM": _u("1", "image stem convs (ResNet 7x7, Inception Conv2d_1a, VGG first layer) on the MFMA stem kernels"),
    "KUNGFU_LINEAR_WGRAD": _u("1", "linear-layer weight gradients on the split-K MFMA kernel"),
    "KUNGFU_DEV_KNOBS": _u("0", "1: honour the dev (A/B) knobs below"),
    "KUNGFU_SELF_SPEC": _l("this worker's host:port"),
    "KUNGFU_INIT_PEERS": _l("initial peer list"),
    "KUNGFU_INIT_RUNNERS": _l("initial runner list"),
    "KUNGFU_INIT_CLUSTER_VERSION": _l("initial cluster version"),
    "KUNGFU_PARENT_ID": _l("runner that started this worker"),
    "KUNGFU_CONFIG_SERVER": _l("elastic config server URL"),
    "KUNGFU_JOB_START_TIMESTAMP": _l("job start time"),
    "KUNGFU_PROC_START_TIMESTAMP": _l("worker start time"),
    "KUNGFU_HIP_DEVICE_ORDINAL": _l("the worker's HIP device"),
    "KUNGFU_HIP_VISIBLE_DEVICES": _l("devices assigned to the worker (-isolate-gpus)"),
    "KUNGFU_ALLOW_XGMI": _l("several workers may share a GPU (-allow-xgmi)"),
    "KUNGFU_SELF_IP": _l("this worker's IP (single mode)"),
    "KUNGFU_CONV_TILE_RULES": _d("2", "1 = the round-2 conv tile defaults"),
    "KUNGFU_WGRAD_PLAN": _d("2", "1: the round-5 weight-gradient plan rules (tile variant, row-image kernel, split counts)"),
    "KUNGFU_CONV_T224": _d("1", "0: no 224x256 conv tiles (one- or two-round grids of 256x256 tiles keep them)"),
    "KUNGFU_CONV_ROWS": _d("1", "0: stride-1 3x3 convs with Cin = Cout = 64 on the tap-wise kernel, not the row-image one"),
    "KUNGFU_VGG_FUSED": _d("1", "VGG-16 conv/ReLU/pool stack as one autograd node (0: the per-layer modules)"),
    "KUNGFU_GRAPH_MULTIRANK": _u("1", "0: GraphedStep keeps multi-rank RCCL steps eager (capture uses the comm stream as origin)"),
}

RETIRED: Dict[str, str] = {
    "KUNGFU_LINEAR_GEMM": "linear layers on gemm.hip measured slower than hipBLASLt (r4_gemm_nt.md)",
    "KUNGFU_LINEAR_WGRAD_ATOMICS": "atomic split-K linear wgrad measured 3 % slower (r4t29)",
    "KUNGFU_GELU_FWD": "the one-exponential GELU forward measured 0.6 % slower (r4t20)",
    "KUNGFU_WGRAD_STREAM": "weight gradients on a side stream measured 1.2 % slower (r3)",
    "KUNGFU_BN_INLAUNCH_FIN": "the path is removed: BN finalize inside the conv launch measured 0.55 (r3) and 1.2 (r6) ms/step slower",
    "KUNGFU_CONV_PRIO": "s_setprio in the conv tiles measured neutral (r3)",
    "KUNGFU_STEM_FUSED_BWD": "the one-pass fused stem backward measured slower (r3)",
    "KUNGFU_COMM_STREAM_PRIORITY": "a high-priority comm stream measured 2x slower (r1)",
    "KUNGFU_BN_SKIP_FINALIZE": "timing-only experiment (wrong numerics), retired",
    "KUNGFU_BERT_GEMM": "unused",
    "KUNGFU_CONV_STAGGER": "the measured winner is the only path: on (+0.8 %, r3)",
    "KUNGFU_CONV_PERSIST_BLOCKS": "the measured winner is the only path: 4 persistent blocks per CU",
    "KUNGFU_WGRAD_STAGGER": "the measured winner is the only path: on for 256x256 tiles only (r3)",
    "KUNGFU_WROWS_STAGGER": "the measured winner is the only path: on (r3)",
    "KUNGFU_WGRAD_KB32": "the measured winner is the only path: off (r4t1)",
    "KUNGFU_BN_NT": "the measured winner is the only path: non-temporal loads (r3f)",
    "KUNGFU_BN_MAXGRID": "the measured winner is the only path: the kernel default grid",
    "KUNGFU_ATTN_BWD_WAVES": "the measured winner is the only path: 8 waves (r4t15)",
    "KUNGFU_BN_CONCAT": "the measured winner is the only path: on (module attribute ops.fused_bn.CONCAT_ENABLED)",
    "KUNGFU_BN_BATCH_FIN": "the measured winner is the only path: on (r4t25; module attribute ops.fused_bn._BATCH_FIN)",
    "KUNGFU_LN_BIAS_LINK": "the measured winner is the only path: on (module attribute ops.layernorm._BIAS_LINK)",
    "KUNGFU_GELU_BIAS_LINK": "the measured winner is the only path: on (module attribute ops.linear._GELU_LINK)",
    "KUNGFU_RESIDUAL_LINK": "the measured winner is the only path: on (r4t14; module attribute ops.linear._RES_LINK)",
    "KUNGFU_LINEAR_DIRECT_WGRAD": "the measured winner is the only path: on (module attribute ops.linear._DIRECT_WGRAD)",
    "KUNGFU_FUSED_XENT": "the measured winner is the only path: on (r4t22; module attribute ops.xent._ENABLED)",
    "KUNGFU_PAIR_NATIVE": "the measured winner is the only path: the native prefetch thread (r4t22)",
    "KUNGFU_GRAPH_SEGMENTED": "the whole-graph N-rank layout is gone: N-rank capture is always segmented (r6)",
}

MACROS = ("KUNGFU_DISABLE_TRACE", "KUNGFU_ENABLE_TRACE", "KUNGFU_AMD_CAPI_H", "KUNGFU_ENABLE_HIP")

PREFIXES = ("KUNGFU_RCCL_MIN_CTAS_", "KUNGFU_RCCL_MAX_CTAS_")


def dev_enabled() -> bool:
    return os.environ.get("KUNGFU_DEV_KNOBS", "0") not in ("", "0")


def get(name: str, default: Optional[str] = None) -> Optional[str]:
    k = KNOBS.get(name)
    if k is None:
        raise KeyError("unregistered knob %s (add it to kungfu_amd/knobs.py)" % name)
    dflt = default if default is not None else k.default
    if k.kind == "dev" and not dev_enabled():
        return dflt
    return os.environ.get(name, dflt)


def get_int(name: str, default: Optional[int] = None) -> int:
    v = get(name, None if default is None else str(default))
    return int(v) if v not in (None, "") else 0


_checked = [False]


def check_environ(environ=None) -> list:
    env = os.environ if environ is None else environ
    msgs = []
    for name in sorted(env):
        if not name.startswith("KUNGFU_"):
            continue
        if name in KNOBS:
            if KNOBS[name].kind == "dev" and not (env.get("KUNGFU_DEV_KNOBS", "0") not in ("", "0")):
                msgs.append("%s is a developer A/B knob and is IGNORED without KUNGFU_DEV_KNOBS=1" % name)
            continue
        if name.startswith(PREFIXES):
            continue
        if name in RETIRED:
            msgs.append("%s is retired and has no effect: %s" % (name, RETIRED[name]))
            continue
        close = difflib.get_close_matches(name, list(KNOBS), n=1, cutoff=0.75)
        msgs.append("unknown setting %s%s (see kungfu_amd/knobs.py)" % (
            name, " -- did you mean %s?" % close[0] if close else ""))
    for m in msgs:
        warnings.warn("kungfu_amd: " + m, KnobWarning, stacklevel=3)
    return msgs


def check_environ_once() -> None:
    if not _checked[0]:
        _checked[0] = True
        check_environ()


def table() -> str:
    heads = {"user": "Configuration", "dev": "Developer A/B switches (need KUNGFU_DEV_KNOBS=1)",
             "test": "Test hooks", "launcher": "Worker environment set by the launcher (not set by hand)"}
    out = []
    for kind in ("user", "dev", "test", "launcher"):
        rows = ["## %s" % heads[kind], "", "| variable | default | meaning |", "|---|---|---|"]
        for n, k in KNOBS.items():
            if k.kind == kind:
                rows.append("| `%s` | %s | %s |" % (n, "" if k.default is None else "`%s`" % k.default, k.doc))
        out.append("\n".join(rows))
    rows = ["## Retired (setting one only warns)", "", "| variable | why |", "|---|---|"]
    rows += ["| `%s` | %s |" % (n, why) for n, why in RETIRED.items()]
    out.append("\n".join(rows))
    return "\n\n".join(out) + "\n"
```

### kungfu_amd/ops/fused_block.py

```python
from __future__ import annotations

import os
from typing import List, Optional

import torch
import torch.nn.functional as F

from .._lib import buf_ok, hip, hip_available
from ..parallel.mixed import deliver, direct_target, shadow

_ENABLED = os.environ.get("KUNGFU_FUSED_BLOCK", "1") != "0"


_CAPTURE = None


def _capture(bn, kind, dz, x, mean, invstd, gate, dg, db):
    _CAPTURE.append(dict(bn=bn, kind=kind, dz=dz.detach().clone(), x=x.detach().clone(), mean=mean.clone(),
                         invstd=invstd.clone(), gate=None if gate is None else gate.clone(),
                         dg=dg.detach().clone(), db=db.detach().clone()))


def set_enabled(on: bool) -> bool:
    global _ENABLED
    old, _ENABLED = _ENABLED, bool(on)
    return old


def _cl(t: torch.Tensor) -> torch.Tensor:
    return t if t.is_contiguous(memory_format=torch.channels_last) else t.contiguous(memory_format=torch.channels_last)


def _sums(bn, dev) -> torch.Tensor:
    ws = getattr(bn, "_kf_sums", None)
    if ws is None or ws.device != dev:
        ws = torch.zeros(hip().conv_stat_slots * 2 * bn.num_features, dtype=torch.float64, device=dev)
        bn._kf_sums = ws
    return ws


def _wgrad(dy, x, w, stride, pad):
    from .conv import wgrad

    return wgrad(dy, x, w, stride, pad)


class _FlipCache:

    def __init__(self, space):
        self.space = space
        self.index = {}
        self.gen = -1

    def register(self, i: int, w: torch.Tensor):
        if i not in self.index:
            co, ci, kh, kw = w.shape
            self.index[i] = torch.empty((ci, co, kh, kw), dtype=torch.bfloat16, device=w.device).contiguous(
                memory_format=torch.channels_last)
            self.gen = -1

    def get(self, i: int) -> torch.Tensor:
        if self.gen != self.space.shadow_gen:
            idx = sorted(self.index)
            ws = [self.space.shadow_view(j) for j in idx]
            ws = [w if w.dim() == 4 else w.view(w.shape[0], w.shape[1], 1, 1) for w in ws]
            hip().conv_flip_weights(ws, [self.index[j] for j in idx])
            self.gen = self.space.shadow_gen
        return self.index[i]


def _flip_cache(space) -> _FlipCache:
    c = getattr(space, "_kf_flip", None)
    if c is None:
        c = space._kf_flip = _FlipCache(space)
    return c


def _dgrad(dy, x, w, stride, pad, out: Optional[torch.Tensor] = None, flipped: Optional[torch.Tensor] = None,
           bn=None, out_mask: Optional[torch.Tensor] = None, acc_even: bool = False):
    H = hip()
    wt = flipped if flipped is not None else None
    if stride == 1:
        wt = wt if wt is not None else H.conv_flip_weight(w)
        _dgrad.fused = bn is not None
        if bn is not None:
            ws, bx, fc, mk = bn
            return H.conv(dy, wt, 1, ws, out, -1, bx, fc, mk, acc_mask=out_mask, acc_even=acc_even)
        return H.conv(dy, wt, 1, None, out, acc_mask=out_mask, acc_even=acc_even)
    assert out_mask is None and not acc_even
    ks = w.shape[2]
    if stride == 2 and out is None and _even_s2(x, dy, ks):
        wt = wt if wt is not None else H.conv_flip_weight(w)
        if ks == 3 and bn is not None:
            ws, bx, fc, mk = bn
            _dgrad.fused = True
            return H.conv_dgrad_s2(dy, wt, 3, ws, bx, fc, mk)
        _dgrad.fused = False
        dx = H.conv_dgrad_s2(dy, wt, ks)
        if ks == 1:
            dx.view(dx.shape[0], dx.shape[1], dx.shape[2] // 2, 2, dx.shape[3] // 2, 2)[:, :, :, 1:, :, :].zero_()
            dx.view(dx.shape[0], dx.shape[1], dx.shape[2] // 2, 2, dx.shape[3] // 2, 2)[:, :, :, 0, :, 1:].zero_()
        return dx
    _dgrad.fused = False
    dx = torch.ops.aten.convolution_backward(dy, x, w, None, [stride, stride], [pad, pad], [1, 1], False, [0, 0], 1,
                                             [True, False, False])[0]
    if out is not None:
        out.add_(dx)
        return out
    return _cl(dx)


def _even_s2(x, dy, ks) -> bool:
    return (x.shape[2] == 2 * dy.shape[2] and x.shape[3] == 2 * dy.shape[3] and ks in (1, 3)
            and hip().conv_supported(dy.shape[1], x.shape[1], ks, 1))


def _dgrad_s2_even(dy, x, w, flipped=None):
    H = hip()
    wt = flipped if flipped is not None else H.conv_flip_weight(w)
    return H.conv_dgrad_s2(dy, wt, 1)


class _TailSlot:
    __slots__ = ("ws", "y3", "mask", "ready", "dx_ptr")

    def __init__(self, ws, y3, mask):
        self.ws, self.y3, self.mask = ws, y3, mask
        self.ready = False
        self.dx_ptr = 0


class _Spec:
    __slots__ = ("bns", "stride", "ds", "dtypes", "direct", "wsrc")

    def __init__(self, bns, stride, ds):
        self.bns, self.stride, self.ds = bns, stride, ds
        self.dtypes = None
        self.direct = None
        self.wsrc = None


class _BottleneckFn(torch.autograd.Function):
    @staticmethod
    def forward(ctx, spec: _Spec, x, *params):
        H = hip()
        dev = x.device
        ws = [p for p in params]
        ws_bf = [w if w.dtype == torch.bfloat16 else w.to(torch.bfloat16) for w in ws[0::3]]
        ws_bf = [_cl(w) for w in ws_bf]
        gam, bet = ws[1::3], ws[2::3]
        s = spec.stride
        outs = []

        def bn(i, y, res, relu, res_coef=None, apply=True):
            m = spec.bns[i]
            return H.bn_forward(y, res, gam[i], bet[i], m.running_mean, m.running_var, m.momentum, m.eps, True, relu,
                                m.num_batches_tracked, _sums(m, dev), res_coef=res_coef, apply=apply)

        def conv(i, inp, w_, st_):
            return H.conv(inp, w_, st_, _sums(spec.bns[i], dev))

        y1 = conv(0, x, ws_bf[0], 1)
        z1, m1, i1, c1, _ = bn(0, y1, None, True)
        y2 = conv(1, z1, ws_bf[1], s)
        z2, m2, i2, c2, _ = bn(1, y2, None, True)
        y3 = conv(2, z2, ws_bf[2], 1)
        if spec.ds:
            yd = conv(3, x, ws_bf[3], s)
            _, md, idd, cd, _ = bn(3, yd, None, False, apply=False)
            out, m3, i3, c3, mask3 = bn(2, y3, yd, True, res_coef=cd)
        else:
            yd = md = idd = cd = None
            out, m3, i3, c3, mask3 = bn(2, y3, x, True)
        ctx.prev = getattr(x, "_kf_tail", None)
        ctx.tail = _TailSlot(_sums(spec.bns[2], dev), y3, mask3)
        ctx.spec = spec
        ctx.wdtypes = [w.dtype for w in ws[0::3]]
        ctx.save_for_backward(x, y1, z1, y2, z2, y3, yd, *ws_bf, *gam, m1, i1, c1, m2, i2, c2, m3, i3, c3, mask3,
                              md, idd, cd)
        return out

    @staticmethod
    def backward(ctx, dout):
        H = hip()
        spec = ctx.spec
        nb = 4 if spec.ds else 3
        t = list(ctx.saved_tensors)
        x, y1, z1, y2, z2, y3, yd = t[:7]
        w = t[7:7 + nb]
        g = t[7 + nb:7 + 2 * nb]
        (m1, i1, c1, m2, i2, c2, m3, i3, c3, mask3, md, idd, cd) = t[7 + 2 * nb:]
        s = spec.stride
        dout = _cl(dout)
        fl = [None] * nb
        if spec.wsrc is not None:
            for k, src in enumerate(spec.wsrc):
                if src is not None:
                    fl[k] = src[0].get(src[1])
        dbn = [None] * nb
        dw = [None] * nb
        wgrad = _wgrad

        ws = [_sums(b, dout.device) for b in spec.bns]
        tail = ctx.tail
        use3 = tail.ready and dout.data_ptr() == tail.dx_ptr
        if tail.ready and not use3:
            tail.ws.zero_()
        tail.ready, tail.y3, tail.mask = False, None, None
        in_place = use3 and not spec.ds
        dy3, didt, dg3, db3 = H.bn_backward(dout, y3, m3, i3, g[2], c3, mask3, True, True, not in_place,
                                            ws[2] if use3 else None, dres_x=yd if spec.ds else None,
                                            dres_sums=ws[3] if spec.ds else None)
        dbn[2] = (dg3, db3)
        if _CAPTURE is not None:
            _capture(spec.bns[2], "mask", dout, y3, m3, i3, mask3, dg3, db3)
        dz2 = _dgrad(dy3, z2, w[2], 1, 0, flipped=fl[2], bn=(ws[1], y2, c2, None))
        dw[2] = wgrad(dy3, z2, w[2], 1, 0)
        dy2, _, dg2, db2 = H.bn_backward(dz2, y2, m2, i2, g[1], c2, None, True, True, False, ws[1])
        dbn[1] = (dg2, db2)
        if _CAPTURE is not None:
            _capture(spec.bns[1], "relu", dz2, y2, m2, i2, c2, dg2, db2)
        dz1 = _dgrad(dy2, z1, w[1], s, 1, flipped=fl[1], bn=(ws[0], y1, c1, None))
        fused1 = _dgrad.fused
        dw[1] = wgrad(dy2, z1, w[1], s, 1)
        dy1, _, dg1, db1 = H.bn_backward(dz1, y1, m1, i1, g[0], c1, None, True, True, False,
                                         ws[0] if fused1 else None)
        dbn[0] = (dg1, db1)
        if _CAPTURE is not None:
            _capture(spec.bns[0], "relu", dz1, y1, m1, i1, c1, dg1, db1)
        acc_even = False
        if spec.ds:
            dyd, _, dgd, dbd = H.bn_backward(didt, yd, md, idd, g[3], cd, None, False, True, False, ws[3])
            dbn[3] = (dgd, dbd)
            if _CAPTURE is not None:
                _capture(spec.bns[3], "plain", didt, yd, md, idd, None, dgd, dbd)
            if s == 2 and _even_s2(x, dyd, 1):
                dx = _dgrad_s2_even(dyd, x, w[3], flipped=fl[3])
                acc_even = True
            else:
                dx = _dgrad(dyd, x, w[3], s, 0, flipped=fl[3])
            dw[3] = wgrad(dyd, x, w[3], s, 0)
        elif in_place:
            dx = dout
        else:
            dx = didt
        om = mask3 if in_place else None
        prev = ctx.prev
        if prev is not None and prev.y3 is not None and prev.y3.shape == dx.shape:
            dx = _dgrad(dy1, x, w[0], 1, 0, out=dx, flipped=fl[0], bn=(prev.ws, prev.y3, None, prev.mask),
                        out_mask=om, acc_even=acc_even)
            prev.ready, prev.dx_ptr = True, dx.data_ptr()
        else:
            dx = _dgrad(dy1, x, w[0], 1, 0, out=dx, flipped=fl[0], out_mask=om, acc_even=acc_even)
        dw[0] = wgrad(dy1, x, w[0], 1, 0)
        grads: List[Optional[torch.Tensor]] = []
        for i in range(nb):
            gw = dw[i]
            if gw.dtype != ctx.wdtypes[i]:
                gw = gw.to(ctx.wdtypes[i])
            dgm, dbt = dbn[i]
            tgt = spec.direct[i] if spec.direct is not None else None
            if tgt is not None:
                deliver(tgt[0], dgm)
                deliver(tgt[1], dbt)
                dgm = dbt = None
            grads += [gw, dgm, dbt]
        return (None, dx, *grads)


def eligible(block, x: torch.Tensor) -> bool:
    if not (_ENABLED and block.training and x.is_cuda and x.dtype == torch.bfloat16 and x.dim() == 4):
        return False
    if not x.is_contiguous(memory_format=torch.channels_last) or not hip_available():
        return False
    widest = max(block.conv1.in_channels, block.conv3.out_channels, block.conv1.out_channels)
    if not buf_ok(x.numel() // x.shape[1] * widest):
        return False
    H = hip()
    convs = [block.conv1, block.conv2, block.conv3] + ([block.downsample[0]] if block.downsample is not None else [])
    for c in convs:
        if c.bias is not None or c.groups != 1 or c.dilation != (1, 1):
            return False
        if not H.conv_supported(c.in_channels, c.out_channels, c.kernel_size[0], c.stride[0]):
            return False
    if block.conv2.kernel_size != (3, 3) or block.conv2.padding != (1, 1):
        return False
    if block.downsample is not None and block.downsample[0].kernel_size != (1, 1):
        return False
    bns = [block.bn1, block.bn2, block.bn3] + ([block.downsample[1]] if block.downsample is not None else [])
    for b in bns:
        if not (b.track_running_stats and b.momentum is not None and b.affine):
            return False
        if not H.bn_supported_channels(b.num_features):
            return False
    return True


def bottleneck_forward(block, x: torch.Tensor) -> torch.Tensor:
    ds = block.downsample is not None
    convs = [block.conv1, block.conv2, block.conv3] + ([block.downsample[0]] if ds else [])
    bns = [block.bn1, block.bn2, block.bn3] + ([block.downsample[1]] if ds else [])
    spec = getattr(block, "_kf_spec", None)
    if spec is None or spec.ds != ds:
        spec = _Spec(bns, block.conv2.stride[0], ds)
        block._kf_spec = spec
    params = []
    direct = []
    wsrc = []
    for c, b in zip(convs, bns):
        w = shadow(c.weight)
        params += [w, b.weight, b.bias]
        tw, tb = direct_target(b.weight), direct_target(b.bias)
        direct.append((tw, tb) if tw is not None and tb is not None else None)
        tc = direct_target(c.weight)
        if tc is not None and w is not c.weight and w.dtype == torch.bfloat16:
            fc = _flip_cache(tc[0])
            fc.register(tc[1], w)
            wsrc.append((fc, tc[1]))
        else:
            wsrc.append(None)
    spec.direct = direct if any(d is not None for d in direct) else None
    spec.wsrc = wsrc if any(v is not None for v in wsrc) else None
    out = _BottleneckFn.apply(spec, x, *params)
    if out.grad_fn is not None:
        out._kf_tail = out.grad_fn.tail
    return out
```

Baseline: 12790.

## Fold BN stat finalize into apply kernels with last-block workspace release

Adds a fold mode in which each block of the BN forward and backward apply kernels recomputes the per-channel finalize from the f64 slot sums into shared memory. This removes the separate finalize launch for the bottleneck BNs. The last block, tracked by an atomic counter, zeroes the sums workspace. A launch rule picks the folded path only when the redundant per-block prologue reads stay small relative to payload bytes, capping the grid at 512. It is enabled by default through a new knob and adds a per-BN counter tensor. The trade-off is redundant sum reads in every block, plus possibly fewer blocks when the grid is capped.

After: 12850 (median of 6 runs). No clear change (+0.4%).

```diff
diff --git a/csrc/kernels/bind_bn.cpp b/csrc/kernels/bind_bn.cpp
--- a/csrc/kernels/bind_bn.cpp
+++ b/csrc/kernels/bind_bn.cpp
@@ -98,10 +98,18 @@
     return out;
 }
 
+int *fold_ctr_ptr(const OptTensor &o, const char *op, const Dev &dev, bool with_sums) {
+    if (!has(o)) return nullptr;
+    TORCH_CHECK(with_sums, op, ": fold_ctr must come with sums (it belongs to that workspace)");
+    check_dense(*o, op, "fold_ctr", dev, at::kInt, 1);
+    return o->data_ptr<int>();
+}
+
 std::vector<at::Tensor> bn_forward(at::Tensor x, OptTensor res, at::Tensor weight, at::Tensor bias,
                                    OptTensor running_mean, OptTensor running_var, double momentum, double eps,
                                    bool training, bool relu, OptTensor num_batches, OptTensor sums, OptTensor res_coef,
-                                   bool apply, OptTensor out, c10::optional<std::vector<at::Tensor>> pre) {
+                                   bool apply, OptTensor out, c10::optional<std::vector<at::Tensor>> pre,
+                                   OptTensor fold_ctr) {
     const char *op = "bn_forward";
     auto sh = bn_shape(x, op);
     const int C = sh.channels;
@@ -137,6 +145,7 @@
         check_dense((*pre)[2], op, "pre[2]", dev, at::kFloat, 2 * C);
     }
     double *sp = training ? stats_ptr(sums, op, C, dev, "sums") : nullptr;
+    int *fc = fold_ctr_ptr(fold_ctr, op, dev, has(sums));
 
     c10::DeviceGuard gd(x.device());
     auto fopt = x.options().dtype(at::kFloat);
@@ -155,13 +164,13 @@
                            training, b.rm, b.rv, static_cast<float>(momentum), static_cast<float>(eps),
                            partial.defined() ? partial.data_ptr<float>() : nullptr, mean.data_ptr<float>(),
                            invstd.data_ptr<float>(), coef.data_ptr<float>(), b.nbt, stream_of(x, 0), sp, rc, apply, y_ld,
-                           prefin);
+                           prefin, fc);
     return {y, mean, invstd, coef, mask};
 }
 
 std::vector<at::Tensor> bn_backward(at::Tensor dy, at::Tensor x, at::Tensor mean, at::Tensor invstd, at::Tensor weight,
                                     at::Tensor fcoef, OptTensor mask, bool relu, bool training, bool want_dres,
-                                    OptTensor sums, OptTensor dres_x, OptTensor dres_sums) {
+                                    OptTensor sums, OptTensor dres_x, OptTensor dres_sums, OptTensor fold_ctr) {
     const char *op = "bn_backward";
     auto sh = bn_shape(x, op);
     const int C = sh.channels;
@@ -177,6 +186,7 @@
         mp = mask->data_ptr<uint8_t>();
     }
     double *sp = stats_ptr(sums, op, C, dev, "sums");
+    int *fc = fold_ctr_ptr(fold_ctr, op, dev, sp != nullptr);
     const uint16_t *dsx = nullptr;
     double *dsp = nullptr;
     if (has(dres_x)) {
@@ -200,7 +210,7 @@
                             invstd.data_ptr<float>(), weight.data_ptr<float>(), sh, relu, training,
                             partial.defined() ? partial.data_ptr<float>() : nullptr, dw.data_ptr<float>(),
                             db.data_ptr<float>(), coef.data_ptr<float>(), bf16_mut(dx),
-                            want_dres ? bf16_mut(dres) : nullptr, stream_of(x, 0), sp, dsx, dsp, dy_ld);
+                            want_dres ? bf16_mut(dres) : nullptr, stream_of(x, 0), sp, dsx, dsp, dy_ld, 0, fc);
     return {dx, dres, dw, db};
 }
 
@@ -336,7 +346,8 @@
           py::arg("res"), py::arg("weight"), py::arg("bias"), py::arg("running_mean"), py::arg("running_var"),
           py::arg("momentum"), py::arg("eps"), py::arg("training"), py::arg("relu"),
           py::arg("num_batches") = py::none(), py::arg("sums") = py::none(), py::arg("res_coef") = py::none(),
-          py::arg("apply") = true, py::arg("out") = py::none(), py::arg("pre") = py::none());
+          py::arg("apply") = true, py::arg("out") = py::none(), py::arg("pre") = py::none(),
+          py::arg("fold_ctr") = py::none());
     m.def("bn_backward_multi", &bn_backward_multi,
           "backward of several BN+ReLUs (slices of one concatenation's gradient): one batched finalize");
     m.def("bn_finalize_multi", &bn_finalize_multi,
@@ -344,7 +355,30 @@
     m.def("bn_backward", &bn_backward, "fused NHWC BN(+residual)(+ReLU) backward -> (dx, dres, dweight, dbias)",
           py::arg("dy"), py::arg("x"), py::arg("mean"), py::arg("invstd"), py::arg("weight"), py::arg("fcoef"),
           py::arg("mask"), py::arg("relu"), py::arg("training"), py::arg("want_dres"), py::arg("sums") = py::none(),
-          py::arg("dres_x") = py::none(), py::arg("dres_sums") = py::none());
+          py::arg("dres_x") = py::none(), py::arg("dres_sums") = py::none(), py::arg("fold_ctr") = py::none());
+    m.def(
+        "bn_fold_rule",
+        [](c10::optional<double> max_ratio, c10::optional<int64_t> grid) {
+            const kfk::BnFoldRule old = kfk::bn_fold_rule();
+            kfk::BnFoldRule r = old;
+            if (max_ratio) r.max_ratio = static_cast<float>(*max_ratio);
+            if (grid) r.grid = narrow(*grid, "bn_fold_rule", "grid");
+            TORCH_CHECK(r.max_ratio >= 0 && r.grid >= 1, "bn_fold_rule: max_ratio must be >= 0, grid >= 1");
+            kfk::set_bn_fold_rule(r);
+            return std::make_pair(static_cast<double>(old.max_ratio), static_cast<int64_t>(old.grid));
+        },
+        "the fold mode's launch rule (max prologue / payload byte ratio, grid cap); sets what is given -> the old pair",
+        py::arg("max_ratio") = py::none(), py::arg("grid") = py::none());
+    m.def(
+        "bn_fold_grid",
+        [](int64_t rows, int64_t C, int64_t streams, bool keep_grid) {
+            const char *op = "bn_fold_grid";
+            const int c = narrow(C, op, "C");
+            TORCH_CHECK(kfk::bn_supported_channels(c) && rows >= 1, op, ": unsupported shape");
+            return kfk::bn_fold_grid(kfk::BNShape{rows, c}, narrow(streams, op, "streams"), keep_grid);
+        },
+        "grid of the folded apply launch for [rows, C] moving `streams` 16-byte vectors per vector, 0 = separate finalize",
+        py::arg("rows"), py::arg("C"), py::arg("streams"), py::arg("keep_grid") = false);
     m.def("bn_pool_supported", [](int64_t C, int64_t H, int64_t W) {
         const char *op = "bn_pool_supported";
         return kfk::bn_pool_supported(kfk::BNShape{H * W, narrow(C, op, "C")}, narrow(H, op, "H"), narrow(W, op, "W"));
diff --git a/csrc/kernels/bn.hip b/csrc/kernels/bn.hip
--- a/csrc/kernels/bn.hip
+++ b/csrc/kernels/bn.hip
@@ -4,6 +4,7 @@
 
 #include <cstdlib>
 #include <stdexcept>
+#include <type_traits>
 
 namespace kfk {
 
@@ -214,25 +215,9 @@
     if (c >= C) return;
     const float g = gamma ? gamma[c] : 1.f, b = beta ? beta[c] : 0.f;
     const float rm = run_mean ? run_mean[c] : 0.f, rv = run_mean ? run_var[c] : 0.f;
-    const double *sp = sums + c;
-    double vs[kStatSlots], vq[kStatSlots];
-#pragma unroll
-    for (int k = 0; k < kStatSlots; ++k) {
-        vs[k] = sp[k * 2 * C];
-        vq[k] = sp[k * 2 * C + C];
-    }
-    double s = 0, q = 0;
-#pragma unroll
-    for (int k = 0; k < kStatSlots; ++k) {
-        s += vs[k];
-        q += vq[k];
-    }
-    double *zp = sums + c;
-#pragma unroll
-    for (int k = 0; k < kStatSlots; ++k) {
-        zp[k * 2 * C] = 0.0;
-        zp[k * 2 * C + C] = 0.0;
-    }
+    double s, q;
+    bn_fin_slot_sums<kStatSlots>(sums, c, C, s, q);
+    bn_fin_slot_zero<kStatSlots>(sums, c, C);
     bn_fin_fwd_channel(c, C, s, q, rows, g, b, rm, rv, mean, invstd, run_mean, run_var, momentum, eps, coef);
 }
 
@@ -244,25 +229,9 @@
     const int C = d.C;
     const float g = d.gamma ? d.gamma[c] : 1.f, bb = d.beta ? d.beta[c] : 0.f;
     const float rm = d.run_mean ? d.run_mean[c] : 0.f, rv = d.run_mean ? d.run_var[c] : 0.f;
-    const double *sp = d.sums + c;
-    double vs[kStatSlots], vq[kStatSlots];
-#pragma unroll
-    for (int k = 0; k < kStatSlots; ++k) {
-        vs[k] = sp[k * 2 * C];
-        vq[k] = sp[k * 2 * C + C];
-    }
-    double s = 0, q = 0;
-#pragma unroll
-    for (int k = 0; k < kStatSlots; ++k) {
-        s += vs[k];
-        q += vq[k];
-    }
-    double *zp = d.sums + c;
-#pragma unroll
-    for (int k = 0; k < kStatSlots; ++k) {
-        zp[k * 2 * C] = 0.0;
-        zp[k * 2 * C + C] = 0.0;
-    }
+    double s, q;
+    bn_fin_slot_sums<kStatSlots>(d.sums, c, C, s, q);
+    bn_fin_slot_zero<kStatSlots>(d.sums, c, C);
     bn_fin_fwd_channel(c, C, s, q, d.rows, g, bb, rm, rv, d.mean, d.invstd, d.run_mean, d.run_var, d.momentum, d.eps,
                        d.coef);
 }
@@ -280,16 +249,87 @@
 }
 
 
-template <int CVEC, bool RES, bool RELU, bool RESC = false, bool SOUT = false>
+struct BnFoldFwd {
+    double *sums = nullptr;
+    int *ctr = nullptr;
+    int64_t rows = 0;
+    const float *gamma = nullptr, *beta = nullptr;
+    float *mean = nullptr, *invstd = nullptr, *run_mean = nullptr, *run_var = nullptr, *coef = nullptr;
+    int64_t *num_batches = nullptr;
+    float momentum = 0.f, eps = 0.f;
+};
+
+struct BnFoldBwd {
+    double *sums = nullptr;
+    int *ctr = nullptr;
+    int64_t rows = 0;
+    const float *gamma = nullptr, *mean = nullptr, *invstd = nullptr;
+    float *dgamma = nullptr, *dbeta = nullptr, *coef = nullptr;
+    bool training = true;
+};
+
+template <int CVEC>
+__device__ __forceinline__ void bn_fold_fwd(const BnFoldFwd &fa, float *lcoef) {
+    constexpr int C = CVEC * 8;
+    const bool lead = blockIdx.x == 0;
+    if (fa.num_batches && lead && threadIdx.x == 0) fa.num_batches[0] += 1;
+    for (int c = threadIdx.x; c < C; c += bn_threads<CVEC>()) {
+        const float g = fa.gamma ? fa.gamma[c] : 1.f, b = fa.beta ? fa.beta[c] : 0.f;
+        const bool run = lead && fa.run_mean;
+        const float rm = run ? fa.run_mean[c] : 0.f, rv = run ? fa.run_var[c] : 0.f;
+        double s, q;
+        bn_fin_slot_sums<kStatSlots>(fa.sums, c, C, s, q);
+        const BnFwdVals v = bn_fin_fwd_values(s, q, fa.rows, g, b, rm, rv, run, fa.momentum, fa.eps);
+        lcoef[c] = v.scale;
+        lcoef[C + c] = v.shift;
+        if (lead) bn_fin_fwd_store(c, C, v, fa.mean, fa.invstd, fa.run_mean, fa.run_var, fa.coef);
+    }
+    __syncthreads();
+}
+
+template <int CVEC>
+__device__ __forceinline__ void bn_fold_bwd(const BnFoldBwd &fa, float *lcoef) {
+    constexpr int C = CVEC * 8;
+    const bool lead = blockIdx.x == 0;
+    for (int c = threadIdx.x; c < C; c += bn_threads<CVEC>()) {
+        const float g = fa.gamma ? fa.gamma[c] : 1.f, mu = fa.mean[c], is = fa.invstd[c];
+        double s0, s1;
+        bn_fin_slot_sums<kStatSlots>(fa.sums, c, C, s0, s1);
+        const BnBwdVals v = bn_fin_bwd_values(s0, s1, fa.rows, g, mu, is, fa.training);
+        lcoef[c] = v.k1;
+        lcoef[C + c] = v.k2;
+        lcoef[2 * C + c] = v.k3;
+        if (lead) bn_fin_bwd_store(c, C, v, fa.dgamma, fa.dbeta, fa.coef);
+    }
+    __syncthreads();
+}
+
+template <int CVEC>
+__device__ __forceinline__ void bn_fold_release(double *__restrict__ sums, int *ctr) {
+    __shared__ int last;
+    if (threadIdx.x == 0) last = atomicAdd(ctr, 1) == static_cast<int>(gridDim.x) - 1;
+    __syncthreads();
+    if (!last) return;
+    for (int i = threadIdx.x; i < kStatSlots * 2 * CVEC * 8; i += bn_threads<CVEC>()) sums[i] = 0.0;
+    if (threadIdx.x == 0) atomicExch(ctr, 0);
+}
+
+
+template <int CVEC, bool RES, bool RELU, bool RESC = false, bool SOUT = false, bool FOLD = false>
 __global__ __launch_bounds__(kBlock) void bn_apply_kernel(const uint4 *__restrict__ x, const uint4 *__restrict__ res,
                                                           const float *__restrict__ coef, uint4 *__restrict__ y,
                                                           uint8_t *__restrict__ mask, int64_t nvec,
                                                           const float *__restrict__ rcoef = nullptr, int ntm = 0,
-                                                          int64_t y_ldv = 0) {
+                                                          int64_t y_ldv = 0, BnFoldFwd fa = {}) {
     constexpr int C = CVEC * 8;
     const bool ntl = ntm & 1, nts = ntm & 2;
     const int64_t tid = static_cast<int64_t>(blockIdx.x) * bn_threads<CVEC>() + threadIdx.x;
     const int cv = static_cast<int>(tid % CVEC);
+    __shared__ float lcoef[FOLD ? 2 * C : 1];
+    if constexpr (FOLD) {
+        bn_fold_fwd<CVEC>(fa, lcoef);
+        coef = lcoef;
+    }
     float sc[8], sh[8], rsc[8], rsh[8];
 #pragma unroll
     for (int k = 0; k < 8; ++k) {
@@ -337,6 +377,7 @@
             if (RES && RELU) mask[i] = static_cast<uint8_t>(m);
         }
     }
+    if constexpr (FOLD) bn_fold_release<CVEC>(fa.sums, fa.ctr);
 }
 
 
@@ -662,41 +703,31 @@
     const int c = blockIdx.x * blockDim.x + threadIdx.x;
     if (c >= C) return;
     const float g = gamma ? gamma[c] : 1.f, mu = mean[c], is = invstd[c];
-    const double *sp = sums + c;
-    double v0[kStatSlots], v1[kStatSlots];
-#pragma unroll
-    for (int k = 0; k < kStatSlots; ++k) {
-        v0[k] = sp[k * 2 * C];
-        v1[k] = sp[k * 2 * C + C];
-    }
-    double s0 = 0, s1 = 0;
-#pragma unroll
-    for (int k = 0; k < kStatSlots; ++k) {
-        s0 += v0[k];
-        s1 += v1[k];
-    }
-    double *zp = sums + c;
-#pragma unroll
-    for (int k = 0; k < kStatSlots; ++k) {
-        zp[k * 2 * C] = 0.0;
-        zp[k * 2 * C + C] = 0.0;
-    }
+    double s0, s1;
+    bn_fin_slot_sums<kStatSlots>(sums, c, C, s0, s1);
+    bn_fin_slot_zero<kStatSlots>(sums, c, C);
     bn_fin_bwd_channel(c, C, s0, s1, rows, g, mu, is, dgamma, dbeta, coef, training);
 }
 
 
-template <int CVEC, int RM, bool DRES, class G>
+template <int CVEC, int RM, bool DRES, class G, bool FOLD = false>
 __global__ __launch_bounds__(kBlock) void bn_bwd_apply_kernel(G grad, const uint4 *__restrict__ x,
                                                               const float *__restrict__ fcoef,
                                                               const uint8_t *__restrict__ mask,
                                                               const float *__restrict__ coef, uint4 *__restrict__ dx,
                                                               uint4 *__restrict__ dres, int64_t nvec,
                                                               const uint4 *__restrict__ dsx = nullptr,
-                                                              double *__restrict__ dsums = nullptr, int ntm = 0) {
+                                                              double *__restrict__ dsums = nullptr, int ntm = 0,
+                                                              BnFoldBwd fa = {}) {
     constexpr int C = CVEC * 8;
     const bool ntl = ntm & 1, nts = ntm & 2;
     const int64_t tid = static_cast<int64_t>(blockIdx.x) * bn_threads<CVEC>() + threadIdx.x;
     const int cv = static_cast<int>(tid % CVEC);
+    __shared__ float lcoef[FOLD ? 3 * C : 1];
+    if constexpr (FOLD) {
+        bn_fold_bwd<CVEC>(fa, lcoef);
+        coef = lcoef;
+    }
     float k1[8], k2[8], k3[8], sc[8], sh[8];
 #pragma unroll
     for (int k = 0; k < 8; ++k) {
@@ -773,6 +804,7 @@
             atomicAdd(sl + C + c, a2);
         }
     }
+    if constexpr (FOLD) bn_fold_release<CVEC>(fa.sums, fa.ctr);
 }
 
 template <typename F>
@@ -805,6 +837,16 @@
     return static_cast<int>(g);
 }
 
+BnFoldRule g_fold_rule{0.03f, 512};
+
+int fold_grid(int64_t nvec, int cvec, int streams, bool keep_grid) {
+    int g = apply_grid(nvec, cvec);
+    if (!keep_grid && g > g_fold_rule.grid) g = g_fold_rule.grid;
+    const double payload = static_cast<double>(nvec) * 16.0 * streams;
+    const double prologue = static_cast<double>(g) * kStatSlots * 2.0 * cvec * 8 * sizeof(double);
+    return prologue <= g_fold_rule.max_ratio * payload ? g : 0;
+}
+
 void launch_stats(const uint16_t *x, BNShape sh, const float *gamma, const float *beta, float *run_mean,
                   float *run_var, float momentum, float eps, float *partial, float *mean, float *invstd, float *coef,
                   int64_t *num_batches, hipStream_t s) {
@@ -825,12 +867,17 @@
                           const float *invstd, const float *gamma, BNShape sh, int rm, bool training, float *partial,
                           float *dgamma, float *dbeta, float *coef, uint16_t *dx, uint16_t *dres, hipStream_t s,
                           double *sums = nullptr, const uint16_t *dres_x = nullptr, double *dres_sums = nullptr,
-                          int phase = 0) {
+                          int phase = 0, int *fold_ctr = nullptr) {
     const int C = sh.channels, cvec = C / 8;
     const int64_t nvec = sh.rows * cvec;
     Chunking ch = chunking(sh);
     const uint4 *xx = reinterpret_cast<const uint4 *>(x);
-    if (phase == 2) {
+    int fg = 0;
+    if constexpr (std::is_same<G, DirectGrad>::value) {
+        if (sums && fold_ctr && phase == 0 && rm != RM_NONE)
+            fg = fold_grid(nvec, cvec, 3 + (dres ? 1 : 0) + (dres && dres_x ? 1 : 0), dres && dres_x);
+    }
+    if (phase == 2 || fg) {
     } else if (sums) {
         bn_bwd_finalize_sums<<<(C + 255) / 256, 256, 0, s>>>(sums, C, sh.rows, gamma, mean, invstd, dgamma, dbeta,
                                                              coef, training);
@@ -852,13 +899,26 @@
                                                                    invstd, dgamma, dbeta, coef, training);
     }
     if (phase == 3) return;
-    const int g = apply_grid(nvec, cvec);
+    const int g = fg ? fg : apply_grid(nvec, cvec);
     uint4 *o = reinterpret_cast<uint4 *>(dx), *r = reinterpret_cast<uint4 *>(dres);
     dispatch_cvec(cvec, [&](auto cvc) {
         constexpr int CV = decltype(cvc)::value;
         auto go = [&](auto rmc, auto drc) {
             constexpr int RM = decltype(rmc)::value;
             constexpr bool DR = decltype(drc)::value;
+            if constexpr (std::is_same<G, DirectGrad>::value && RM != RM_NONE) {
+                if (fg) {
+                    BnFoldBwd fa;
+                    fa.sums = sums, fa.ctr = fold_ctr, fa.rows = sh.rows;
+                    fa.gamma = gamma, fa.mean = mean, fa.invstd = invstd;
+                    fa.dgamma = dgamma, fa.dbeta = dbeta, fa.coef = coef, fa.training = training;
+                    bn_bwd_apply_kernel<CV, RM, DR, G, true><<<g, bn_threads<CV>(), 0, s>>>(
+                        grad, xx, fcoef, mask, coef, o, r, nvec,
+                        DR ? reinterpret_cast<const uint4 *>(dres_x) : nullptr, DR ? dres_sums : nullptr,
+                        bn_nt_mode(), fa);
+                    return;
+                }
+            }
             bn_bwd_apply_kernel<CV, RM, DR, G><<<g, bn_threads<CV>(), 0, s>>>(
                 grad, xx, fcoef, mask, coef, o, r, nvec, DR ? reinterpret_cast<const uint4 *>(dres_x) : nullptr,
                 DR ? dres_sums : nullptr, bn_nt_mode());
@@ -909,16 +969,27 @@
 
 int bn_num_chunks(BNShape sh) { return chunking(sh).nchunks; }
 
+BnFoldRule bn_fold_rule() { return g_fold_rule; }
+void set_bn_fold_rule(BnFoldRule r) { g_fold_rule = r; }
+int bn_fold_grid(BNShape sh, int streams, bool keep_grid) {
+    return fold_grid(sh.rows * (sh.channels / 8), sh.channels / 8, streams, keep_grid);
+}
+
 void launch_bn_forward(const uint16_t *x, const uint16_t *res, const float *gamma, const float *beta, uint16_t *y,
                        uint8_t *mask, BNShape sh, bool relu, bool training, float *run_mean, float *run_var,
                        float momentum, float eps, float *partial, float *mean, float *invstd, float *coef,
                        int64_t *num_batches, hipStream_t s, double *sums, const float *res_coef, bool apply,
-                       int64_t y_ld, bool prefinalized) {
+                       int64_t y_ld, bool prefinalized, int *fold_ctr) {
     const int C = sh.channels, cvec = C / 8;
     if (y_ld > 0 && (y_ld % 8 || y_ld < C || res || !relu))
         throw std::invalid_argument("bn_forward: a strided output needs BN+ReLU without residual, row stride % 8");
     const int64_t nvec = sh.rows * cvec;
-    if (training && sums) {
+    const bool sout = y_ld > 0 && y_ld != C;
+    const int fg = training && sums && fold_ctr && apply && !prefinalized && !sout
+                       ? fold_grid(nvec, cvec, res ? 3 : 2, false)
+                       : 0;
+    if (fg) {
+    } else if (training && sums) {
         if (!prefinalized)
             bn_sums_finalize<<<(C + 255) / 256, 256, 0, s>>>(sums, C, sh.rows, gamma, beta, mean, invstd, run_mean,
                                                              run_var, momentum, eps, coef, num_batches);
@@ -929,7 +1000,7 @@
         bn_eval_coef<<<(C + 255) / 256, 256, 0, s>>>(C, gamma, beta, run_mean, run_var, eps, mean, invstd, coef);
     }
     if (!apply) return;
-    const int g = apply_grid(nvec, cvec);
+    const int g = fg ? fg : apply_grid(nvec, cvec);
     const int ntm = bn_nt_mode();
     dispatch_cvec(cvec, [&](auto cvc) {
         constexpr int CV = decltype(cvc)::value;
@@ -937,7 +1008,21 @@
         const uint4 *xv = reinterpret_cast<const uint4 *>(x);
         const uint4 *rv = reinterpret_cast<const uint4 *>(res);
         uint4 *yv = reinterpret_cast<uint4 *>(y);
-        if (res && res_coef) {
+        if (fg) {
+            BnFoldFwd fa;
+            fa.sums = sums, fa.ctr = fold_ctr, fa.rows = sh.rows, fa.gamma = gamma, fa.beta = beta;
+            fa.mean = mean, fa.invstd = invstd, fa.run_mean = run_mean, fa.run_var = run_var, fa.coef = coef;
+            fa.num_batches = num_batches, fa.momentum = momentum, fa.eps = eps;
+            auto go = [&](auto rs, auto rl, auto rc) {
+                bn_apply_kernel<CV, decltype(rs)::value, decltype(rl)::value, decltype(rc)::value, false, true>
+                    <<<g, NT, 0, s>>>(xv, rv, coef, yv, mask, nvec, res_coef, ntm, 0, fa);
+            };
+            using T = std::true_type;
+            using F = std::false_type;
+            if (res && res_coef) relu ? go(T(), T(), T()) : go(T(), F(), T());
+            else if (res) relu ? go(T(), T(), F()) : go(T(), F(), F());
+            else relu ? go(F(), T(), F()) : go(F(), F(), F());
+        } else if (res && res_coef) {
             if (relu) bn_apply_kernel<CV, true, true, true><<<g, NT, 0, s>>>(xv, rv, coef, yv, mask, nvec, res_coef, ntm);
             else bn_apply_kernel<CV, true, false, true><<<g, NT, 0, s>>>(xv, rv, coef, yv, mask, nvec, res_coef, ntm);
         } else if (res) {
@@ -957,7 +1042,7 @@
                         const float *mean, const float *invstd, const float *gamma, BNShape sh, bool relu,
                         bool training, float *partial, float *dgamma, float *dbeta, float *coef, uint16_t *dx,
                         uint16_t *dres, hipStream_t s, double *sums, const uint16_t *dres_x, double *dres_sums,
-                        int64_t dy_ld, int phase) {
+                        int64_t dy_ld, int phase, int *fold_ctr) {
     const int rm = !relu ? RM_NONE : (mask ? RM_BITS : RM_COEF);
     if (dy_ld > 0 && dy_ld != sh.channels) {
         if (dy_ld % 8) throw std::invalid_argument("bn_backward: dy row stride must be a multiple of 8");
@@ -967,7 +1052,7 @@
         return;
     }
     launch_backward_impl(DirectGrad{reinterpret_cast<const uint4 *>(dy), (bn_nt_mode() & 1) != 0}, x, fcoef, mask, mean, invstd, gamma, sh, rm,
-                         training, partial, dgamma, dbeta, coef, dx, dres, s, sums, dres_x, dres_sums, phase);
+                         training, partial, dgamma, dbeta, coef, dx, dres, s, sums, dres_x, dres_sums, phase, fold_ctr);
 }
 
 bool bn_pool_supported(BNShape sh, int H, int W) {
diff --git a/csrc/kernels/bn_fin.hpp b/csrc/kernels/bn_fin.hpp
--- a/csrc/kernels/bn_fin.hpp
+++ b/csrc/kernels/bn_fin.hpp
@@ -6,43 +6,116 @@
 
 namespace kfk {
 
+template <int NSLOT>
+__device__ __forceinline__ void bn_fin_slot_sums(const double *__restrict__ sums, int c, int C, double &s0,
+                                                 double &s1) {
+    const double *sp = sums + c;
+    double v0[NSLOT], v1[NSLOT];
+#pragma unroll
+    for (int k = 0; k < NSLOT; ++k) {
+        v0[k] = sp[k * 2 * C];
+        v1[k] = sp[k * 2 * C + C];
+    }
+    s0 = 0, s1 = 0;
+#pragma unroll
+    for (int k = 0; k < NSLOT; ++k) {
+        s0 += v0[k];
+        s1 += v1[k];
+    }
+}
+
+template <int NSLOT>
+__device__ __forceinline__ void bn_fin_slot_zero(double *__restrict__ sums, int c, int C) {
+    double *zp = sums + c;
+#pragma unroll
+    for (int k = 0; k < NSLOT; ++k) {
+        zp[k * 2 * C] = 0.0;
+        zp[k * 2 * C + C] = 0.0;
+    }
+}
+
+struct BnFwdVals {
+    float mean, invstd, run_mean, run_var, scale, shift;
+};
+
+__device__ __forceinline__ BnFwdVals bn_fin_fwd_values(double s, double q, int64_t rows, float g, float b, float rm,
+                                                       float rv, bool running, float momentum, float eps) {
+    const float nz = -(eps * 0.f);
+    BnFwdVals v;
+    const double m = s / rows;
+    double var = fma(-m, m, q / rows);
+    if (var < 0) var = 0;
+    const float is = rsqrtf(static_cast<float>(var) + eps);
+    const float sc = g * is;
+    v.mean = static_cast<float>(m);
+    v.invstd = is;
+    v.run_mean = v.run_var = 0.f;
+    if (running) {
+        const double unbiased = rows > 1 ? var * rows / (rows - 1) : var;
+        v.run_mean = fmaf(1.f - momentum, rm, nz) + fmaf(momentum, static_cast<float>(m), nz);
+        v.run_var = fmaf(1.f - momentum, rv, nz) + fmaf(momentum, static_cast<float>(unbiased), nz);
+    }
+    v.scale = sc;
+    v.shift = fmaf(-static_cast<float>(m), sc, b);
+    return v;
+}
+
+__device__ __forceinline__ void bn_fin_fwd_store(int c, int C, const BnFwdVals &v, float *mean, float *invstd,
+                                                 float *run_mean, float *run_var, float *coef) {
+    mean[c] = v.mean;
+    invstd[c] = v.invstd;
+    if (run_mean) {
+        run_mean[c] = v.run_mean;
+        run_var[c] = v.run_var;
+    }
+    coef[c] = v.scale;
+    coef[C + c] = v.shift;
+}
+
 __device__ __forceinline__ void bn_fin_fwd_channel(int c, int C, double s, double q, int64_t rows, float g, float b,
                                                    float rm, float rv, float *mean, float *invstd, float *run_mean,
                                                    float *run_var, float momentum, float eps, float *coef) {
-    const double m = s / rows;
-    double var = q / rows - m * m;
-    if (var < 0) var = 0;
-    const float is = rsqrtf(static_cast<float>(var) + eps);
-    const float sc = g * is;
-    mean[c] = static_cast<float>(m);
-    invstd[c] = is;
-    if (run_mean) {
-        const double unbiased = rows > 1 ? var * rows / (rows - 1) : var;
-        run_mean[c] = (1.f - momentum) * rm + momentum * static_cast<float>(m);
-        run_var[c] = (1.f - momentum) * rv + momentum * static_cast<float>(unbiased);
+    bn_fin_fwd_store(c, C, bn_fin_fwd_values(s, q, rows, g, b, rm, rv, run_mean != nullptr, momentum, eps), mean,
+                     invstd, run_mean, run_var, coef);
+}
+
+struct BnBwdVals {
+    float dgamma, dbeta, k1, k2, k3;
+};
+
+__device__ __forceinline__ BnBwdVals bn_fin_bwd_values(double s0, double s1, int64_t rows, float g, float mu,
+                                                       float is, bool training) {
+    BnBwdVals v;
+    const double db = s0, dg = static_cast<double>(is) * fma(-static_cast<double>(mu), db, s1);
+    v.dgamma = static_cast<float>(dg);
+    v.dbeta = static_cast<float>(db);
+    const float a = g * is;
+    v.k1 = a;
+    if (training) {
+        const float inv_m = 1.f / static_cast<float>(rows);
+        const float k2 = -a * static_cast<float>(dg) * is * inv_m;
+        v.k2 = k2;
+        v.k3 = fmaf(-k2, mu, -a * static_cast<float>(db) * inv_m);
+    } else {
+        v.k2 = 0.f;
+        v.k3 = 0.f;
     }
-    coef[c] = sc;
-    coef[C + c] = b - static_cast<float>(m) * sc;
+    return v;
+}
+
+__device__ __forceinline__ void bn_fin_bwd_store(int c, int C, const BnBwdVals &v, float *dgamma, float *dbeta,
+                                                 float *coef) {
+    dgamma[c] = v.dgamma;
+    dbeta[c] = v.dbeta;
+    coef[c] = v.k1;
+    coef[C + c] = v.k2;
+    coef[2 * C + c] = v.k3;
 }
 
 __device__ __forceinline__ void bn_fin_bwd_channel(int c, int C, double s0, double s1, int64_t rows, float g,
                                                    float mu, float is, float *dgamma, float *dbeta, float *coef,
                                                    bool training) {
-    const double db = s0, dg = static_cast<double>(is) * (s1 - static_cast<double>(mu) * db);
-    dgamma[c] = static_cast<float>(dg);
-    dbeta[c] = static_cast<float>(db);
-    const float a = g * is;
-    if (training) {
-        const float inv_m = 1.f / static_cast<float>(rows);
-        const float k2 = -a * static_cast<float>(dg) * is * inv_m;
-        coef[c] = a;
-        coef[C + c] = k2;
-        coef[2 * C + c] = -a * static_cast<float>(db) * inv_m - k2 * mu;
-    } else {
-        coef[c] = a;
-        coef[C + c] = 0.f;
-        coef[2 * C + c] = 0.f;
-    }
+    bn_fin_bwd_store(c, C, bn_fin_bwd_values(s0, s1, rows, g, mu, is, training), dgamma, dbeta, coef);
 }
 
 }
diff --git a/csrc/kernels/kernels.hpp b/csrc/kernels/kernels.hpp
--- a/csrc/kernels/kernels.hpp
+++ b/csrc/kernels/kernels.hpp
@@ -242,16 +242,24 @@
 };
 void launch_bn_bwd_finalize_multi(const BnBwdFinBatch &b, hipStream_t s);
 
+struct BnFoldRule {
+    float max_ratio;
+    int grid;
+};
+BnFoldRule bn_fold_rule();
+void set_bn_fold_rule(BnFoldRule r);
+int bn_fold_grid(BNShape sh, int streams, bool keep_grid);
+
 void launch_bn_forward(const uint16_t *x, const uint16_t *res, const float *gamma, const float *beta, uint16_t *y,
                        uint8_t *mask, BNShape sh, bool relu, bool training, float *run_mean, float *run_var,
                        float momentum, float eps, float *partial, float *mean, float *invstd, float *coef,
                        int64_t *num_batches, hipStream_t s, double *sums = nullptr, const float *res_coef = nullptr,
-                       bool apply = true, int64_t y_ld = 0, bool prefinalized = false);
+                       bool apply = true, int64_t y_ld = 0, bool prefinalized = false, int *fold_ctr = nullptr);
 void launch_bn_backward(const uint16_t *dy, const uint16_t *x, const float *fcoef, const uint8_t *mask,
                         const float *mean, const float *invstd, const float *gamma, BNShape sh, bool relu,
                         bool training, float *partial, float *dgamma, float *dbeta, float *coef, uint16_t *dx,
                         uint16_t *dres, hipStream_t s, double *sums = nullptr, const uint16_t *dres_x = nullptr,
-                        double *dres_sums = nullptr, int64_t dy_ld = 0, int phase = 0);
+                        double *dres_sums = nullptr, int64_t dy_ld = 0, int phase = 0, int *fold_ctr = nullptr);
 
 inline int pool_out(int h) { return (h + 2 - 3) / 2 + 1; }
 bool bn_pool_supported(BNShape sh, int H, int W);
diff --git a/kungfu_amd/knobs.py b/kungfu_amd/knobs.py
--- a/kungfu_amd/knobs.py
+++ b/kungfu_amd/knobs.py
@@ -92,6 +92,7 @@
     "KUNGFU_CONV_T224": _d("1", "0: no 224x256 conv tiles (one- or two-round grids of 256x256 tiles keep them)"),
     "KUNGFU_CONV_ROWS": _d("1", "0: stride-1 3x3 convs with Cin = Cout = 64 on the tap-wise kernel, not the row-image one"),
     "KUNGFU_VGG_FUSED": _d("1", "VGG-16 conv/ReLU/pool stack as one autograd node (0: the per-layer modules)"),
+    "KUNGFU_BN_FOLD": _d("1", "0: the bottleneck BNs keep a finalize launch of their own (1: folded into the apply kernels where the launch rule selects the shape)"),
     "KUNGFU_GRAPH_MULTIRANK": _u("1", "0: GraphedStep keeps multi-rank RCCL steps eager (capture uses the comm stream as origin)"),
 }
 
diff --git a/kungfu_amd/ops/fused_block.py b/kungfu_amd/ops/fused_block.py
--- a/kungfu_amd/ops/fused_block.py
+++ b/kungfu_amd/ops/fused_block.py
@@ -6,10 +6,12 @@
 import torch
 import torch.nn.functional as F
 
+from .. import knobs
 from .._lib import buf_ok, hip, hip_available
 from ..parallel.mixed import deliver, direct_target, shadow
 
 _ENABLED = os.environ.get("KUNGFU_FUSED_BLOCK", "1") != "0"
+_BN_FOLD = knobs.get("KUNGFU_BN_FOLD") != "0"
 
 
 _CAPTURE = None
@@ -24,6 +26,12 @@
 def set_enabled(on: bool) -> bool:
     global _ENABLED
     old, _ENABLED = _ENABLED, bool(on)
+    return old
+
+
+def set_bn_fold(on: bool) -> bool:
+    global _BN_FOLD
+    old, _BN_FOLD = _BN_FOLD, bool(on)
     return old
 
 
@@ -37,6 +45,16 @@
         ws = torch.zeros(hip().conv_stat_slots * 2 * bn.num_features, dtype=torch.float64, device=dev)
         bn._kf_sums = ws
     return ws
+
+
+def _fold_ctr(bn, dev) -> Optional[torch.Tensor]:
+    if not _BN_FOLD:
+        return None
+    ctr = getattr(bn, "_kf_fold_ctr", None)
+    if ctr is None or ctr.device != dev:
+        ctr = torch.zeros(1, dtype=torch.int32, device=dev)
+        bn._kf_fold_ctr = ctr
+    return ctr
 
 
 def _wgrad(dy, x, w, stride, pad):
@@ -155,7 +173,8 @@
         def bn(i, y, res, relu, res_coef=None, apply=True):
             m = spec.bns[i]
             return H.bn_forward(y, res, gam[i], bet[i], m.running_mean, m.running_var, m.momentum, m.eps, True, relu,
-                                m.num_batches_tracked, _sums(m, dev), res_coef=res_coef, apply=apply)
+                                m.num_batches_tracked, _sums(m, dev), res_coef=res_coef, apply=apply,
+                                fold_ctr=_fold_ctr(m, dev) if apply else None)
 
         def conv(i, inp, w_, st_):
             return H.conv(inp, w_, st_, _sums(spec.bns[i], dev))
@@ -202,6 +221,7 @@
         wgrad = _wgrad
 
         ws = [_sums(b, dout.device) for b in spec.bns]
+        fc = [_fold_ctr(b, dout.device) for b in spec.bns[:3]]
         tail = ctx.tail
         use3 = tail.ready and dout.data_ptr() == tail.dx_ptr
         if tail.ready and not use3:
@@ -210,13 +230,14 @@
         in_place = use3 and not spec.ds
         dy3, didt, dg3, db3 = H.bn_backward(dout, y3, m3, i3, g[2], c3, mask3, True, True, not in_place,
                                             ws[2] if use3 else None, dres_x=yd if spec.ds else None,
-                                            dres_sums=ws[3] if spec.ds else None)
+                                            dres_sums=ws[3] if spec.ds else None, fold_ctr=fc[2] if use3 else None)
         dbn[2] = (dg3, db3)
         if _CAPTURE is not None:
             _capture(spec.bns[2], "mask", dout, y3, m3, i3, mask3, dg3, db3)
         dz2 = _dgrad(dy3, z2, w[2], 1, 0, flipped=fl[2], bn=(ws[1], y2, c2, None))
         dw[2] = wgrad(dy3, z2, w[2], 1, 0)
-        dy2, _, dg2, db2 = H.bn_backward(dz2, y2, m2, i2, g[1], c2, None, True, True, False, ws[1])
+        dy2, _, dg2, db2 = H.bn_backward(dz2, y2, m2, i2, g[1], c2, None, True, True, False, ws[1],
+                                         fold_ctr=fc[1])
         dbn[1] = (dg2, db2)
         if _CAPTURE is not None:
             _capture(spec.bns[1], "relu", dz2, y2, m2, i2, c2, dg2, db2)
@@ -224,7 +245,7 @@
         fused1 = _dgrad.fused
         dw[1] = wgrad(dy2, z1, w[1], s, 1)
         dy1, _, dg1, db1 = H.bn_backward(dz1, y1, m1, i1, g[0], c1, None, True, True, False,
-                                         ws[0] if fused1 else None)
+                                         ws[0] if fused1 else None, fold_ctr=fc[0] if fused1 else None)
         dbn[0] = (dg1, db1)
         if _CAPTURE is not None:
             _capture(spec.bns[0], "relu", dz1, y1, m1, i1, c1, dg1, db1)
```
